# radoslawkrolikowski/financial-market-data-analysis

Measured on NVIDIA H100. Metric: sequences/sec (train step) biGRU h=256 seq=128 feat=64, higher is better.
Workload: dtype bf16x3 (fp32-class: split bf16 operand pairs on tensor cores, fp32 accumulate / state / gradients)

## Files before the change

### financial_market_data_analysis_b200/_lib.py

```python
from __future__ import annotations

import ctypes as C
import os
import threading

_HERE = os.path.dirname(os.path.abspath(__file__))
LIB_PATH = os.path.join(_HERE, "libbigru_b200.so")

PREC_FP32, PREC_BF16, PREC_BF16X3 = 0, 1, 2
SQNORM_WS = 528
LOSS_CE, LOSS_BCE, LOSS_MLSM = 0, 1, 2
ERR_ARG, ERR_CUDA, ERR_DEVICE, ERR_UNSUPPORTED = -1, -2, -3, -4

_vp, _i, _i64, _f, _u64, _d = C.c_void_p, C.c_int, C.c_int64, C.c_float, C.c_uint64, C.c_double

SIGNATURES = {
    "bigru_last_error": (C.c_char_p, []),
    "bigru_version": (_i, []),
    "bigru_device_check": (_i, [_i]),
    "bigru_plan_create": (_i, [_i, _i, _i, _i, _i, _i, _i, _i, C.POINTER(_vp)]),
    "bigru_plan_destroy": (_i, [_vp]),
    "bigru_param_count": (_i64, [_vp]),
    "bigru_param_offset": (_i, [_vp, _i, _i, _i, C.POINTER(_i64), C.POINTER(_i64), C.POINTER(_i64)]),
    "bigru_workspace_bytes": (_i, [_vp, C.POINTER(C.c_size_t), C.POINTER(C.c_size_t)]),
    "bigru_stash_argmax_offset": (_i, [_vp, C.POINTER(C.c_size_t)]),
    "bigru_stash_output_offset": (_i, [_vp, _i, C.POINTER(C.c_size_t)]),
    "bigru_workspace_region": (_i, [_vp, _i, _i, C.POINTER(_i), C.POINTER(C.c_size_t), C.POINTER(C.c_size_t), C.POINTER(_i64)]),
    "bigru_forward": (_i, [_vp, _vp, _vp, _vp, _f, _i, _i, _u64, _vp, _vp, _vp, _vp, _vp]),
    "bigru_backward": (_i, [_vp, _vp, _vp, _vp, _f, _i, _i, _u64, _vp, _vp, _vp, _vp, _vp, _vp, _vp]),
    "bigru_infer_workspace_bytes": (_i, [_vp, C.POINTER(C.c_size_t)]),
    "bigru_infer": (_i, [_vp, _vp, _vp, _vp, _vp, _vp, _vp]),
    "bigru_forward_lengths": (_i, [_vp, _vp, _vp, _vp, _f, _i, _i, _u64, _vp, _vp, _vp, _vp, _vp, _vp]),
    "bigru_backward_lengths": (_i, [_vp, _vp, _vp, _vp, _f, _i, _i, _u64, _vp, _vp, _vp, _vp, _vp, _vp, _vp, _vp]),
    "bigru_infer_lengths": (_i, [_vp, _vp, _vp, _vp, _vp, _vp, _vp, _vp]),
    "bigru_loss": (_i, [_i, _vp, _vp, _vp, _vp, _i, _i, _d, _vp, _vp, _vp]),
    "bigru_sqnorm": (_i, [_vp, _i64, _vp, _vp, _vp]),
    "bigru_adam_tick": (_i, [_vp, _vp, _vp]),
    "bigru_clip_adam_step_dev": (_i, [_vp, _vp, _vp, _vp, _i64, _vp, _f, _f, _f, _f, _f, _vp, _f, _vp]),
    "bigru_launch_count_add": (None, [C.c_longlong]),
    "bigru_window_gather_norm": (_i, [_vp, _vp, _vp, _i64, _i64, _i, _i, _i, _vp, _vp]),
    "bigru_window_targets": (_i, [_vp, _i64, _i64, _i, _i, _i, _vp, _vp]),
    "bigru_multilabel_counts": (_i, [_vp, _vp, _i, _i, _vp, _vp]),
    "bigru_chunk_minmax": (_i, [_vp, _i64, _i, _i64, _i64, _vp, _vp, _vp]),
    "bigru_infer_window": (_i, [_vp, _vp, _vp, _vp, _i, _i, _i, _i, _i, _i, _i, _vp, _vp, _vp]),
    "bigru_window_features": (_i, [_vp, _vp, _vp, _vp, _vp, _i64, C.POINTER(_i), _i, C.POINTER(_i), _i, C.POINTER(_i), _i, _i, _f, _i,
                                   _f, _f, _vp, _vp, C.POINTER(_i), _vp]),
    "bigru_launch_count": (C.c_longlong, []),
    "bigru_prof_enable": (_i, [_i]),
    "bigru_prof_classes": (_i, []),
    "bigru_prof_class_name": (C.c_char_p, [_i]),
    "bigru_prof_report": (_i, [_i, C.POINTER(_d), C.POINTER(C.c_longlong), C.POINTER(_d), C.POINTER(_d)]),
}

_lib = None
_lock = threading.Lock()


def load():
    global _lib
    with _lock:
        if _lib is None:
            if not os.path.exists(LIB_PATH):
                raise RuntimeError(
                    f"{LIB_PATH} is missing: build it with `python -m financial_market_data_analysis_b200.build` "
                    "(or __graft_entry__.build()). This package has no CPU/PyTorch fallback.")
            lib = C.CDLL(LIB_PATH)
            for name, (res, args) in SIGNATURES.items():
                fn = getattr(lib, name)
                fn.restype, fn.argtypes = res, args
            _lib = lib
    return _lib


def check(rc: int, what: str):
    if rc == 0:
        return
    msg = load().bigru_last_error().decode("utf-8", "replace")
    if rc in (ERR_ARG, ERR_UNSUPPORTED):
        raise ValueError(f"{what}: {msg} (code {rc})")
    raise RuntimeError(f"{what}: {msg} (code {rc})")


def ptr(t):
    return None if t is None else C.c_void_p(t.data_ptr())
```

### financial_market_data_analysis_b200/csrc/api.cu

```cuda
#include "common.cuh"
#include "kernels_f32.cuh"
#include "tc_hopper.cuh"
#include "features.cuh"
#include "infer_small.cuh"

#include <cstring>
#include <new>

static thread_local char g_err[512] = "";
void bigru_set_error(const char* fmt, ...) {
    va_list ap;
    va_start(ap, fmt);
    vsnprintf(g_err, sizeof(g_err), fmt, ap);
    va_end(ap);
}

extern "C" const char* bigru_last_error(void) { return g_err; }
extern "C" int bigru_version(void) { return 207; }

extern "C" int bigru_device_check(int dev) {
    int n = 0;
    if (cudaGetDeviceCount(&n) != cudaSuccess || n <= 0 || dev >= n) {
        cudaGetLastError();
        bigru_set_error("no CUDA device %d (libbigru_b200 has no CPU fallback)", dev);
        return BIGRU_ERR_DEVICE;
    }
    cudaDeviceProp p;
    CUDA_TRY(cudaGetDeviceProperties(&p, dev));
    if (p.major != 9 || p.minor != 0) {
        bigru_set_error("device %d is sm_%d%d; libbigru_b200 is built for sm_90a (H100) only", dev, p.major, p.minor);
        return BIGRU_ERR_DEVICE;
    }
    return BIGRU_OK;
}

struct StashF32 {
    int64_t Y[16], G[16], X[16];
    int64_t YP[16], XP[16];
    int64_t cat, arg, total;
};
struct ScratchF32 {
    int64_t gi, gh, dgi, dgh, dYa, dYb, dhc, dcat, csum, dgiP, dghP, tcw, part, total;
};
static inline int64_t in_pitch(const bigru_plan& p, int l) { return rup(p.in_size(l), 8); }
static inline int64_t plane_floats(const bigru_plan& p, int64_t n) {
    return p.prec == BIGRU_PREC_FP32 ? 0 : rup((p.prec == BIGRU_PREC_BF16X3 ? 2 : 1) * n, 128) / 2;
}
static StashF32 stash_layout(const bigru_plan& p) {
    StashF32 s{};
    int64_t o = 0;
    const int64_t BT = (int64_t)p.B * p.T;
    for (int l = 0; l < p.L; ++l) {
        s.Y[l] = o; o += BT * p.D * p.H;
        s.G[l] = o; o += (int64_t)p.D * BT * 4 * p.H;
        s.X[l] = o; o += BT * p.in_size(l);
        o = rup(o, 64);
        s.YP[l] = o; o += plane_floats(p, BT * p.D * p.H);
        s.XP[l] = o; o += plane_floats(p, BT * in_pitch(p, l));
    }
    s.cat = o; o += (int64_t)p.B * 3 * p.H;
    s.arg = o; o += (int64_t)p.B * p.H;
    s.total = o;
    return s;
}
static int64_t dw_part_floats(const bigru_plan& p, int l, int64_t N) {
    const int64_t BT = (int64_t)p.B * p.T, M = 3LL * p.H;
    const int s = wg_splits(cdiv64(M, htc::WG_BM) * cdiv64(N, htc::WG_BN) * p.D, cdiv64(BT, htc::WG_BK));
    return s > 1 ? (int64_t)s * p.D * M * N : 0;
}
static ScratchF32 scratch_layout(const bigru_plan& p) {
    ScratchF32 s{};
    int64_t o = 0;
    const int64_t BT = (int64_t)p.B * p.T;
    const int64_t wide = p.D * p.H > p.F ? p.D * p.H : p.F;
    s.gi = o; o += (int64_t)p.D * BT * 3 * p.H;
    s.gh = o; o += (int64_t)p.D * p.B * 3 * p.H;
    s.dgi = o; o += (int64_t)p.D * BT * 3 * p.H;
    s.dgh = o; o += (int64_t)p.D * BT * 3 * p.H;
    s.dYa = o; o += BT * wide;
    s.dYb = o; o += BT * wide;
    s.dhc = o; o += (int64_t)p.D * p.B * p.H;
    s.dcat = o; o += (int64_t)p.B * 3 * p.H;
    s.csum = o; o += (int64_t)COLSUM_MAX_CHUNKS * (3 * p.H > p.C ? 3 * p.H : p.C);
    o = rup(o, 64);
    s.dgiP = o; o += plane_floats(p, (int64_t)p.D * BT * 3 * p.H);
    s.dghP = o; o += plane_floats(p, (int64_t)p.D * BT * 3 * p.H);
    s.tcw = o;
    s.part = o;
    if (p.prec != BIGRU_PREC_FP32) {
        const int64_t H3 = 3LL * p.H, B = p.B, C = p.C, D = p.D;
        int64_t need = 0, part = 0;
        for (int l = 0; l < p.L; ++l) {
            const int64_t I = p.in_size(l);
            need = std::max(need, tc_pack_elems(H3, I, D, p.prec));
            need = std::max(need, tc_pack_elems(I, H3, D, p.prec));
            part = std::max(part, std::max(dw_part_floats(p, l, I), dw_part_floats(p, l, p.H)));
        }
        const int64_t h[4] = {tc_gemm_ws_elems(B, C, H3, 1, p.prec), tc_gemm_ws_elems(B, H3, C, 1, p.prec),
                              tc_gemm_ws_elems(C, H3, B, 1, p.prec), tc_gemm_ws_elems(H3, p.H, B, 1, p.prec)};
        for (int64_t v : h) need = std::max(need, v);
        o += plane_floats(p, need);
        s.part = o; o += part;
    }
    s.total = o;
    return s;
}
struct InferF32 {
    int64_t gi, gh, y[2], cat, arg, xp, yp[2], tcw, total;
};
static InferF32 infer_layout(const bigru_plan& p) {
    InferF32 s{};
    int64_t o = 0;
    const int64_t BT = (int64_t)p.B * p.T, DH = (int64_t)p.D * p.H;
    const bool tc = p.prec != BIGRU_PREC_FP32;
    s.gi = o; o += (int64_t)p.D * BT * 3 * p.H;
    s.gh = o; if (!tc) o += (int64_t)p.D * p.B * 3 * p.H;
    s.y[0] = o; o += BT * DH;
    s.y[1] = o; if (!tc && p.L > 1) o += BT * DH;
    s.cat = o; o += (int64_t)p.B * 3 * p.H;
    s.arg = o; o += (int64_t)p.B * p.H;
    o = rup(o, 64);
    s.xp = o; o += plane_floats(p, BT * in_pitch(p, 0));
    s.yp[0] = o; if (p.L > 1) o += plane_floats(p, BT * DH);
    s.yp[1] = o; if (p.L > 2) o += plane_floats(p, BT * DH);
    s.tcw = o;
    if (tc) {
        int64_t need = tc_gemm_ws_elems(p.B, p.C, 3LL * p.H, 1, p.prec);
        for (int l = 0; l < p.L; ++l) need = std::max(need, tc_pack_elems(3LL * p.H, p.in_size(l), p.D, p.prec));
        o += plane_floats(p, need);
    }
    s.total = o;
    return s;
}

static int tc_plan_check(const bigru_plan& p) {
    if (p.prec == BIGRU_PREC_BF16X3 && ((p.H != 128 && p.H != 256) || p.B % 32 != 0)) {
        bigru_set_error("BIGRU_PREC_BF16X3 supports hidden_size 128 or 256 and batch %% 32 == 0 (got H=%d B=%d; the Python mirror pads "
                        "other batch sizes with zero rows); use BIGRU_PREC_FP32 for other shapes", p.H, p.B);
        return BIGRU_ERR_UNSUPPORTED;
    }
    if (p.prec == BIGRU_PREC_BF16 && !(((p.H == 128 || p.H == 256) && p.B % 16 == 0) || (p.H == 512 && p.B % 32 == 0))) {
        bigru_set_error("BIGRU_PREC_BF16 supports hidden_size 128 or 256 with batch %% 16 == 0 and hidden_size 512 with batch %% 32 == 0 "
                        "(got H=%d B=%d; the Python mirror pads other batch sizes with zero rows); use BIGRU_PREC_FP32 for other shapes", p.H, p.B);
        return BIGRU_ERR_UNSUPPORTED;
    }
    return BIGRU_OK;
}

static int plan_gemm(const bigru_plan& p, const GemmArgs& g, int cls, htc::bf16_t* tcw, cudaStream_t st) {
    return p.prec == BIGRU_PREC_FP32 ? sgemm_launch(g, st) : tc_gemm_launch(g, p.prec, cls, tcw, st);
}

static Planes plan_planes(const bigru_plan& p, const float* buf, int64_t off, int64_t cols, int64_t rows, int64_t depth,
                          int64_t pitch) {
    const htc::bf16_t* hi = reinterpret_cast<const htc::bf16_t*>(buf + off);
    return Planes{hi, p.prec == BIGRU_PREC_BF16X3 ? hi + depth * rows * pitch : nullptr, cols, rows, depth, pitch};
}
static Planes input_planes(const bigru_plan& p, const float* planes, int l, bool own) {
    const int64_t BT = (int64_t)p.B * p.T;
    return own ? plan_planes(p, planes, 0, p.in_size(l), BT, 1, in_pitch(p, l))
               : plan_planes(p, planes, 0, (int64_t)p.D * p.H, BT, 1, (int64_t)p.D * p.H);
}
static htc::bf16_t* mut(const Planes& q) { return const_cast<htc::bf16_t*>(q.hi); }
static htc::bf16_t* mut_lo(const Planes& q) { return const_cast<htc::bf16_t*>(q.lo); }

extern "C" int bigru_plan_create(int B, int T, int F, int H, int L, int C, int bidirectional, int precision,
                                 bigru_plan** out) {
    if (!out) { bigru_set_error("plan_create: out is null"); return BIGRU_ERR_ARG; }
    if (B <= 0 || T <= 0 || F <= 0 || H <= 0 || L <= 0 || L > 16 || C <= 0) {
        bigru_set_error("plan_create: bad shape B=%d T=%d F=%d H=%d L=%d C=%d", B, T, F, H, L, C);
        return BIGRU_ERR_ARG;
    }
    if (precision != BIGRU_PREC_FP32 && precision != BIGRU_PREC_BF16 && precision != BIGRU_PREC_BF16X3) {
        bigru_set_error("plan_create: unknown precision %d", precision);
        return BIGRU_ERR_ARG;
    }
    bigru_plan* p = new (std::nothrow) bigru_plan();
    if (!p) { bigru_set_error("plan_create: out of host memory"); return BIGRU_ERR_ARG; }
    p->B = B; p->T = T; p->F = F; p->H = H; p->L = L; p->C = C; p->D = bidirectional ? 2 : 1; p->prec = precision;
    p->nparams = p->off_linb() + C;
    if (precision != BIGRU_PREC_FP32) {
        int rc = tc_plan_check(*p);
        if (rc != BIGRU_OK) { delete p; return rc; }
    }
    p->stash_bytes = (size_t)stash_layout(*p).total * sizeof(float);
    p->scratch_bytes = (size_t)scratch_layout(*p).total * sizeof(float);
    *out = p;
    return BIGRU_OK;
}

extern "C" int bigru_plan_destroy(bigru_plan* plan) { delete plan; return BIGRU_OK; }
extern "C" int64_t bigru_param_count(const bigru_plan* plan) { return plan ? plan->nparams : -1; }

extern "C" int bigru_param_offset(const bigru_plan* p, int layer, int dir, int which, int64_t* offset,
                                  int64_t* rows, int64_t* cols) {
    if (!p || !offset || !rows || !cols || layer < 0 || layer > p->L || dir < 0 || dir >= p->D || which < 0 || which > 3) {
        bigru_set_error("param_offset: bad argument");
        return BIGRU_ERR_ARG;
    }
    if (layer == p->L) {
        if (which == 0) { *offset = p->off_linw(); *rows = p->C; *cols = 3 * p->H; }
        else if (which == 2) { *offset = p->off_linb(); *rows = p->C; *cols = 1; }
        else { bigru_set_error("param_offset: linear has which 0 (weight) or 2 (bias)"); return BIGRU_ERR_ARG; }
        return BIGRU_OK;
    }
    switch (which) {
        case 0: *offset = p->off_wih(layer, dir); *rows = 3 * p->H; *cols = p->in_size(layer); break;
        case 1: *offset = p->off_whh(layer, dir); *rows = 3 * p->H; *cols = p->H; break;
        case 2: *offset = p->off_bih(layer, dir); *rows = 3 * p->H; *cols = 1; break;
        default: *offset = p->off_bhh(layer, dir); *rows = 3 * p->H; *cols = 1; break;
    }
    return BIGRU_OK;
}

extern "C" int bigru_workspace_bytes(const bigru_plan* p, size_t* stash_bytes, size_t* scratch_bytes) {
    if (!p || !stash_bytes || !scratch_bytes) { bigru_set_error("workspace_bytes: null argument"); return BIGRU_ERR_ARG; }
    *stash_bytes = p->stash_bytes;
    *scratch_bytes = p->scratch_bytes;
    return BIGRU_OK;
}

extern "C" int bigru_stash_argmax_offset(const bigru_plan* p, size_t* byte_offset) {
    if (!p || !byte_offset) { bigru_set_error("stash_argmax_offset: null argument"); return BIGRU_ERR_ARG; }
    *byte_offset = (size_t)stash_layout(*p).arg * sizeof(float);
    return BIGRU_OK;
}

extern "C" int bigru_stash_output_offset(const bigru_plan* p, int layer, size_t* byte_offset) {
    if (!p || !byte_offset || layer < 0 || layer >= p->L) { bigru_set_error("stash_output_offset: bad argument"); return BIGRU_ERR_ARG; }
    *byte_offset = (size_t)stash_layout(*p).Y[layer] * sizeof(float);
    return BIGRU_OK;
}

extern "C" int bigru_workspace_region(const bigru_plan* p, int which, int layer, int* in_scratch, size_t* byte_offset,
                                      size_t* lo_byte_offset, int64_t* pitch) {
    if (!p || !in_scratch || !byte_offset || !lo_byte_offset || !pitch) {
        bigru_set_error("workspace_region: null argument");
        return BIGRU_ERR_ARG;
    }
    const bool planes = which == BIGRU_WS_Y_PLANES || which == BIGRU_WS_IN_PLANES || which == BIGRU_WS_DGI_PLANES ||
                        which == BIGRU_WS_DGH_PLANES;
    const bool stashed = which == BIGRU_WS_GATES || which == BIGRU_WS_Y_PLANES || which == BIGRU_WS_IN_PLANES;
    const bool layer_ok = stashed ? layer >= 0 && layer < p->L
                        : which == BIGRU_WS_DY ? layer >= 0 && layer < p->L && layer < 2
                        : which == BIGRU_WS_DCAT ? layer == p->L : layer == 0;
    if (which < 0 || which >= BIGRU_WS_COUNT || !layer_ok) {
        bigru_set_error("workspace_region: bad region %d or layer %d", which, layer);
        return BIGRU_ERR_ARG;
    }
    if (planes && p->prec == BIGRU_PREC_FP32) {
        bigru_set_error("workspace_region: BIGRU_PREC_FP32 keeps no bf16 planes");
        return BIGRU_ERR_UNSUPPORTED;
    }
    const StashF32 S = stash_layout(*p);
    const ScratchF32 W = scratch_layout(*p);
    const int64_t BT = (int64_t)p->B * p->T, H3 = 3LL * p->H, DH = (int64_t)p->D * p->H;
    int64_t off = 0, pt = 0, depth_rows = 0;
    switch (which) {
        case BIGRU_WS_GATES:      off = S.G[layer]; pt = 4LL * p->H; break;
        case BIGRU_WS_Y_PLANES:   off = S.YP[layer]; pt = DH; depth_rows = BT; break;
        case BIGRU_WS_IN_PLANES:  off = S.XP[layer]; pt = in_pitch(*p, layer); depth_rows = BT; break;
        case BIGRU_WS_DGI:        off = W.dgi; pt = H3; break;
        case BIGRU_WS_DGH:        off = W.dgh; pt = H3; break;
        case BIGRU_WS_DGI_PLANES: off = W.dgiP; pt = H3; depth_rows = p->D * BT; break;
        case BIGRU_WS_DGH_PLANES: off = W.dghP; pt = H3; depth_rows = p->D * BT; break;
        case BIGRU_WS_DY:         off = (p->L - 1 - layer) % 2 == 0 ? W.dYa : W.dYb; pt = DH; break;
        case BIGRU_WS_DHC:        off = W.dhc; pt = p->H; break;
        default:                  off = W.dcat; pt = H3; break;
    }
    *in_scratch = stashed ? 0 : 1;
    *byte_offset = (size_t)off * sizeof(float);
    *lo_byte_offset = planes && p->prec == BIGRU_PREC_BF16X3 ? *byte_offset + (size_t)(depth_rows * pt) * 2 : SIZE_MAX;
    *pitch = pt;
    return BIGRU_OK;
}

static inline unsigned nblk(int64_t n, int bs) { return (unsigned)cdiv64(n, bs); }

struct FwdBufs {
    float *gi, *gh, *cat, *arg;
    htc::bf16_t* tcw;
    float *X[16], *Y[16], *G[16], *XP[16], *YP[16];
};
static FwdBufs train_bufs(const bigru_plan& p, float* stash, float* scratch) {
    const StashF32 S = stash_layout(p);
    const ScratchF32 W = scratch_layout(p);
    FwdBufs b{};
    b.gi = scratch + W.gi; b.gh = scratch + W.gh; b.cat = stash + S.cat; b.arg = stash + S.arg;
    b.tcw = reinterpret_cast<htc::bf16_t*>(scratch + W.tcw);
    for (int l = 0; l < p.L; ++l) {
        b.X[l] = stash + S.X[l]; b.Y[l] = stash + S.Y[l]; b.G[l] = stash + S.G[l];
        b.XP[l] = stash + S.XP[l]; b.YP[l] = stash + S.YP[l];
    }
    return b;
}
static FwdBufs infer_bufs(const bigru_plan& p, float* ws) {
    const InferF32 I = infer_layout(p);
    const bool tc = p.prec != BIGRU_PREC_FP32;
    FwdBufs b{};
    b.gi = ws + I.gi; b.gh = ws + I.gh; b.cat = ws + I.cat; b.arg = ws + I.arg;
    b.tcw = reinterpret_cast<htc::bf16_t*>(ws + I.tcw);
    b.XP[0] = ws + I.xp;
    for (int l = 0; l < p.L; ++l) {
        const bool top = l == p.L - 1;
        b.Y[l] = !tc ? ws + I.y[l % 2] : top ? ws + I.y[0] : nullptr;
        b.YP[l] = tc && !top ? ws + I.yp[l % 2] : nullptr;
    }
    return b;
}

static int forward_plan(const bigru_plan& p, const float* params, const float* x, const float* h0, const int* len, float drop,
                        int spatial, int training, uint64_t seed, const FwdBufs& buf, float* logits, float* hn,
                        cudaStream_t st) {
    if (len && h0) {
        bigru_set_error("forward: lengths together with an initial hidden state are not supported");
        return BIGRU_ERR_UNSUPPORTED;
    }
    if (p.prec == BIGRU_PREC_BF16 && h0) {
        bigru_set_error("BIGRU_PREC_BF16: an initial hidden state is not supported; use BIGRU_PREC_FP32 or BIGRU_PREC_BF16X3");
        return BIGRU_ERR_UNSUPPORTED;
    }
    const int B = p.B, T = p.T, H = p.H, D = p.D;
    const int64_t BT = (int64_t)B * T;
    const bool do_drop = training && drop > 0.f;
    const float* inp = x;
    for (int l = 0; l < p.L; ++l) {
        const int I = (int)p.in_size(l);
        if (do_drop && (l == 0 || p.L > 1)) {
            float* xd = buf.X[l];
            KLAUNCH(KC_MISC, 0.0, 0.0, st, dropout_kernel<<<132 * 8, 256, 0, st>>>(inp, xd, BT * I, T, I, l == 0 ? spatial : 0, drop, seed, (uint32_t)l));
            inp = xd;
        }
        float* Y = buf.Y[l];
        float* G = buf.G[l];
        const float* h0l = h0 ? h0 + (int64_t)l * D * B * H : nullptr;
        float* hnl = hn ? hn + (int64_t)l * D * B * H : nullptr;
        if (p.prec != BIGRU_PREC_FP32) {
            const bool own = l == 0 || do_drop;
            const Planes xp = input_planes(p, own ? buf.XP[l] : buf.YP[l - 1], l, own);
            if (own)
                KLAUNCH(KC_PACK, 0.0, 0.0, st, htc::to_planes_kernel<<<132 * 8, 256, 0, st>>>(inp, BT, I, (int)xp.pitch, mut(xp), mut_lo(xp)));
            Planes wp;
            TRY(tc_pack(params + p.off_wih(l, 0), I, 1, p.ld_block(l), 3 * H, I, D, p.prec, buf.tcw, &wp, st));
            {
                ProfScope ps(KC_TC_GEMM, 2.0 * BT * 3 * H * (double)I * D, 0.0, st);
                htc::WgJob j = wg_job(buf.gi, (int)BT, 3 * H, 3 * H, D, cdiv64(I, htc::WG_BK));
                j.bias = params + p.off_bih(l, 0); j.zBias = p.ld_block(l); j.zC = BT * 3 * H;
                j.b.zsel = 1;
                TRY(wg_gemm(j, xp, false, wp, false, p.prec, st));
            }
            htc::bf16_t *yh = nullptr, *yl = nullptr;
            if (buf.YP[l]) {
                const Planes yp = plan_planes(p, buf.YP[l], 0, (int64_t)D * H, BT, 1, (int64_t)D * H);
                yh = mut(yp); yl = mut_lo(yp);
            }
            TRY(tc_scan_fwd(p, l, buf.gi, params + p.off_whh(l, 0), params + p.off_bhh(l, 0), h0l, Y, G, hnl, yh, yl, len, st));
            inp = Y;
            continue;
        }
        GemmArgs g = gemm_args(inp, params + p.off_wih(l, 0), buf.gi, (int)BT, 3 * H, I, I, 1, I, 1, 3 * H);
        g.bias = params + p.off_bih(l, 0);
        g.batch = D; g.zA = 0; g.zB = p.ld_block(l); g.zBias = p.ld_block(l); g.zC = BT * 3 * H;
        TRY(plan_gemm(p, g, KC_TC_GEMM, buf.tcw, st));
        for (int s = 0; s < T; ++s) {
            const float* hp; int64_t sam, zA;
            if (s == 0) { hp = h0l; sam = H; zA = (int64_t)B * H; }
            else {
                hp = Y + (int64_t)(s - 1) * D * H;
                sam = (int64_t)T * D * H;
                zA = D == 2 ? ((int64_t)(T - s) - (s - 1)) * D * H + H : 0;
            }
            GemmArgs r = gemm_args(hp, params + p.off_whh(l, 0), buf.gh, B, 3 * H, hp ? H : 0, sam, 1, H, 1, 3 * H);
            r.bias = params + p.off_bhh(l, 0);
            r.batch = D; r.zA = zA; r.zB = p.ld_block(l); r.zBias = p.ld_block(l); r.zC = (int64_t)B * 3 * H;
            if (hp) { TRY(sgemm_launch(r, st)); }
            else {
                r.A = params; r.K = 1; r.sam = 0; r.sak = 1; r.zA = 0;
                r.mask_period = 1; r.mask_skip = 0;
                TRY(sgemm_launch(r, st));
            }
            KLAUNCH(KC_GATES_FWD, 0.0, 0.0, st, gru_gates_fwd_kernel<<<nblk((int64_t)D * B * H, 256), 256, 0, st>>>(buf.gi, buf.gh, h0l, Y, G,
                                                                              hnl, B, T, H, D, s, len));
        }
        inp = Y;
    }
    KLAUNCH(KC_HEAD, 0.0, 0.0, st, head_pool_kernel<<<nblk((int64_t)B * H, 128), 128, 0, st>>>(buf.Y[p.L - 1], buf.cat, (int*)buf.arg, B, T, H, D, len));
    GemmArgs lin = gemm_args(buf.cat, params + p.off_linw(), logits, B, p.C, 3 * H, 3 * H, 1, 3 * H, 1, p.C);
    lin.bias = params + p.off_linb();
    TRY(plan_gemm(p, lin, KC_HEAD, buf.tcw, st));
    return BIGRU_OK;
}

static int backward_plan(const bigru_plan& p, const float* params, const float* x, const float* h0, const int* len, float drop,
                         int spatial, int training, uint64_t seed, const float* stash, float* scratch,
                         const float* dlogits, float* grads, float* dx, float* dh0, cudaStream_t st) {
    if (len && (h0 || dh0)) {
        bigru_set_error("backward: lengths together with an initial hidden state or its gradient are not supported");
        return BIGRU_ERR_UNSUPPORTED;
    }
    if (p.prec == BIGRU_PREC_BF16 && (h0 || dh0)) {
        bigru_set_error("BIGRU_PREC_BF16: initial hidden state / its gradient are not supported");
        return BIGRU_ERR_UNSUPPORTED;
    }
    const StashF32 S = stash_layout(p);
    const ScratchF32 W = scratch_layout(p);
    const int B = p.B, T = p.T, H = p.H, D = p.D, C = p.C;
    const int64_t BT = (int64_t)B * T, H3 = 3LL * H;
    const bool do_drop = training && drop > 0.f;
    const bool tc = p.prec != BIGRU_PREC_FP32;
    float* dhc = scratch + W.dhc;
    htc::bf16_t* tcw = reinterpret_cast<htc::bf16_t*>(scratch + W.tcw);
    CUDA_TRY(cudaMemsetAsync(grads, 0, sizeof(float) * p.nparams, st));
    GemmArgs a = gemm_args(dlogits, params + p.off_linw(), scratch + W.dcat, B, 3 * H, C, C, 1, 1, 3 * H, 3 * H);
    TRY(plan_gemm(p, a, KC_HEAD, tcw, st));
    GemmArgs w = gemm_args(dlogits, stash + S.cat, grads + p.off_linw(), C, 3 * H, B, 1, C, 1, 3 * H, 3 * H);
    TRY(plan_gemm(p, w, KC_HEAD, tcw, st));
    TRY(colsum_launch(dlogits, grads + p.off_linb(), B, C, C, 1, 0, 0, scratch + W.csum, st));
    KLAUNCH(KC_HEAD, 0.0, 0.0, st, head_bwd_dy_kernel<<<nblk(BT * H, 256), 256, 0, st>>>(scratch + W.dcat, (const int*)(stash + S.arg), scratch + W.dYa, dhc, B, T, H, D, len));
    for (int l = p.L - 1; l >= 0; --l) {
        const int I = (int)p.in_size(l);
        const bool even = (p.L - 1 - l) % 2 == 0;
        const bool drop_l = do_drop && (l == 0 || p.L > 1);
        float* dY = scratch + (even ? W.dYa : W.dYb);
        float* dYnext = scratch + (even ? W.dYb : W.dYa);
        const float* Y = stash + S.Y[l];
        const float* G = stash + S.G[l];
        const float* h0l = h0 ? h0 + (int64_t)l * D * B * H : nullptr;
        float* dgi = scratch + W.dgi;
        float* dgh = scratch + W.dgh;
        if (l != p.L - 1) CUDA_TRY(cudaMemsetAsync(dhc, 0, sizeof(float) * D * B * H, st));
        const Planes gip = plan_planes(p, scratch, W.dgiP, H3, BT, D, H3);
        const Planes ghp = plan_planes(p, scratch, W.dghP, H3, BT, D, H3);
        if (tc) {
            TRY(tc_scan_bwd(p, l, G, Y, h0l, dY, dhc, dgi, dgh, params + p.off_whh(l, 0), mut(gip), mut_lo(gip), mut(ghp), mut_lo(ghp), len, st));
        } else {
            for (int s = 0; s < T; ++s) {
                KLAUNCH(KC_GATES_BWD, 0.0, 0.0, st, gru_gates_bwd_kernel<<<nblk((int64_t)D * B * H, 256), 256, 0, st>>>(G, Y, h0l, dY, dhc, dgi, dgh, B, T, H, D, s, len));
                const int t0 = T - 1 - s, t1 = s;
                GemmArgs r = gemm_args(dgh + (int64_t)t0 * 3 * H, params + p.off_whh(l, 0), dhc, B, H, 3 * H,
                                       (int64_t)T * 3 * H, 1, 1, H, H);
                r.beta = 1; r.batch = D;
                r.zA = BT * 3 * H + (int64_t)(t1 - t0) * 3 * H; r.zB = p.ld_block(l); r.zC = (int64_t)B * H;
                TRY(sgemm_launch(r, st));
            }
        }
        if (dh0) CUDA_TRY(cudaMemcpyAsync(dh0 + (int64_t)l * D * B * H, dhc, sizeof(float) * D * B * H,
                                          cudaMemcpyDeviceToDevice, st));
        if (tc) {
            const int64_t kb = cdiv64(BT, htc::WG_BK);
            float* part = scratch + W.part;
            {
                ProfScope ps(KC_TC_GEMM_DWIH, 2.0 * H3 * I * (double)BT * D, 0.0, st);
                htc::WgJob j = wg_job(grads + p.off_wih(l, 0), (int)H3, I, I, D, kb);
                j.zC = p.ld_block(l); j.a.zsel = 1; j.part = part;
                j.splits = wg_splits(cdiv64(H3, htc::WG_BM) * cdiv64(I, htc::WG_BN) * D, kb);
                const bool own = l == 0 || do_drop;
                TRY(wg_gemm(j, gip, true, input_planes(p, stash + (own ? S.XP[l] : S.YP[l - 1]), l, own), true, p.prec, st));
            }
            if (T > 1) {
                ProfScope ps(KC_TC_GEMM_DWHH, 2.0 * H3 * H * (double)BT * D, 0.0, st);
                htc::WgJob j = wg_job(grads + p.off_whh(l, 0), (int)H3, H, H, D, kb);
                j.zC = p.ld_block(l); j.a.zsel = 1; j.part = part;
                j.b.coff = H; j.b.kshift[0] = -1; j.b.kshift[1] = 1;
                j.splits = wg_splits(cdiv64(H3, htc::WG_BM) * cdiv64(H, htc::WG_BN) * D, kb);
                TRY(wg_gemm(j, ghp, true, plan_planes(p, stash, S.YP[l], (int64_t)D * H, BT, 1, (int64_t)D * H), true, p.prec, st));
            }
        } else {
            const float* inp = drop_l ? stash + S.X[l] : l == 0 ? x : stash + S.Y[l - 1];
            const int splitk = (int)min((int64_t)64, max((int64_t)1, BT / 512));
            for (int d = 0; d < D; ++d) {
                const float* dgi_d = dgi + (int64_t)d * BT * 3 * H;
                const float* dgh_d = dgh + (int64_t)d * BT * 3 * H;
                GemmArgs wi = gemm_args(dgi_d, inp, grads + p.off_wih(l, d), 3 * H, I, (int)BT, 1, 3 * H, 1, I, I);
                wi.splitk = splitk;
                TRY(sgemm_launch(wi, st));
                if (T > 1) {
                    const float* hp = Y + (int64_t)d * H + (d == 0 ? -(int64_t)D * H : (int64_t)D * H);
                    GemmArgs wh = gemm_args(dgh_d, hp, grads + p.off_whh(l, d), 3 * H, H, (int)BT, 1, 3 * H, 1,
                                            (int64_t)D * H, H);
                    wh.splitk = splitk; wh.mask_period = T; wh.mask_skip = d == 0 ? 0 : T - 1;
                    TRY(sgemm_launch(wh, st));
                }
            }
        }
        for (int d = 0; d < D; ++d) {
            const float* dgi_d = dgi + (int64_t)d * BT * 3 * H;
            const float* dgh_d = dgh + (int64_t)d * BT * 3 * H;
            if (h0l) {
                const int tf = d == 0 ? 0 : T - 1;
                GemmArgs w0 = gemm_args(dgh_d + (int64_t)tf * 3 * H, h0l + (int64_t)d * B * H, grads + p.off_whh(l, d),
                                        3 * H, H, B, 1, (int64_t)T * 3 * H, 1, H, H);
                w0.beta = 1;
                TRY(plan_gemm(p, w0, KC_TC_GEMM_DWHH, tcw, st));
            }
            TRY(colsum_launch(dgi_d, grads + p.off_bih(l, d), BT, 3 * H, 3 * H, 1, 0, 0, scratch + W.csum, st));
            TRY(colsum_launch(dgh_d, grads + p.off_bhh(l, d), BT, 3 * H, 3 * H, 1, 0, 0, scratch + W.csum, st));
        }
        float* dxo = l == 0 ? dx : dYnext;
        if (!dxo) continue;
        if (tc) {
            Planes wp;
            TRY(tc_pack(params + p.off_wih(l, 0), 1, I, p.ld_block(l), I, 3 * H, D, p.prec, tcw, &wp, st));
            ProfScope ps(KC_TC_GEMM_DX, 2.0 * BT * I * (double)H3 * D, 0.0, st);
            htc::WgJob j = wg_job(dxo, (int)BT, I, I, 1, D * (H3 / htc::WG_BK));
            j.kbd = (int)(H3 / htc::WG_BK); j.kcat = 1; j.a.zsel = 1; j.b.zsel = 1;
            TRY(wg_gemm(j, gip, false, wp, false, p.prec, st));
        } else {
            for (int d = 0; d < D; ++d) {
                GemmArgs gx = gemm_args(dgi + (int64_t)d * BT * 3 * H, params + p.off_wih(l, d), dxo, (int)BT, I, 3 * H,
                                        3 * H, 1, 1, I, I);
                gx.beta = d;
                TRY(sgemm_launch(gx, st));
            }
        }
        if (drop_l)
            KLAUNCH(KC_MISC, 0.0, 0.0, st, dropout_kernel<<<132 * 8, 256, 0, st>>>(dxo, dxo, BT * I, T, I, l == 0 ? spatial : 0, drop, seed, (uint32_t)l));
    }
    return BIGRU_OK;
}

extern "C" int bigru_forward(const bigru_plan* plan, const float* d_params, const float* d_x, const float* d_h0,
                             float dropout_p, int spatial, int training, uint64_t seed, void* d_stash,
                             void* d_scratch, float* d_logits, float* d_hn, void* stream) {
    return bigru_forward_lengths(plan, d_params, d_x, d_h0, dropout_p, spatial, training, seed, d_stash, d_scratch, d_logits,
                                 d_hn, nullptr, stream);
}

extern "C" int bigru_forward_lengths(const bigru_plan* plan, const float* d_params, const float* d_x, const float* d_h0,
                                     float dropout_p, int spatial, int training, uint64_t seed, void* d_stash,
                                     void* d_scratch, float* d_logits, float* d_hn, const int32_t* d_lengths, void* stream) {
    if (!plan || !d_params || !d_x || !d_stash || !d_scratch || !d_logits) {
        bigru_set_error("forward: null argument");
        return BIGRU_ERR_ARG;
    }
    if (dropout_p < 0.f || dropout_p >= 1.f) { bigru_set_error("forward: dropout_p must be in [0,1)"); return BIGRU_ERR_ARG; }
    return forward_plan(*plan, d_params, d_x, d_h0, d_lengths, dropout_p, spatial, training, seed,
                        train_bufs(*plan, (float*)d_stash, (float*)d_scratch), d_logits, d_hn, (cudaStream_t)stream);
}

extern "C" int bigru_infer_workspace_bytes(const bigru_plan* p, size_t* bytes) {
    if (!p || !bytes) { bigru_set_error("infer_workspace_bytes: null argument"); return BIGRU_ERR_ARG; }
    *bytes = (size_t)infer_layout(*p).total * sizeof(float);
    return BIGRU_OK;
}

extern "C" int bigru_infer(const bigru_plan* plan, const float* d_params, const float* d_x, const float* d_h0,
                           void* d_workspace, float* d_logits, void* stream) {
    return bigru_infer_lengths(plan, d_params, d_x, d_h0, d_workspace, d_logits, nullptr, stream);
}

extern "C" int bigru_infer_lengths(const bigru_plan* plan, const float* d_params, const float* d_x, const float* d_h0,
                                   void* d_workspace, float* d_logits, const int32_t* d_lengths, void* stream) {
    if (!plan || !d_params || !d_x || !d_workspace || !d_logits) {
        bigru_set_error("infer: null argument");
        return BIGRU_ERR_ARG;
    }
    return forward_plan(*plan, d_params, d_x, d_h0, d_lengths, 0.f, 0, 0, 0, infer_bufs(*plan, (float*)d_workspace), d_logits,
                        nullptr, (cudaStream_t)stream);
}

extern "C" int bigru_backward(const bigru_plan* plan, const float* d_params, const float* d_x, const float* d_h0,
                              float dropout_p, int spatial, int training, uint64_t seed, const void* d_stash,
                              void* d_scratch, const float* d_dlogits, float* d_grads, float* d_dx, float* d_dh0,
                              void* stream) {
    return bigru_backward_lengths(plan, d_params, d_x, d_h0, dropout_p, spatial, training, seed, d_stash, d_scratch, d_dlogits,
                                  d_grads, d_dx, d_dh0, nullptr, stream);
}

extern "C" int bigru_backward_lengths(const bigru_plan* plan, const float* d_params, const float* d_x, const float* d_h0,
                                      float dropout_p, int spatial, int training, uint64_t seed, const void* d_stash,
                                      void* d_scratch, const float* d_dlogits, float* d_grads, float* d_dx, float* d_dh0,
                                      const int32_t* d_lengths, void* stream) {
    if (!plan || !d_params || !d_x || !d_stash || !d_scratch || !d_dlogits || !d_grads) {
        bigru_set_error("backward: null argument");
        return BIGRU_ERR_ARG;
    }
    return backward_plan(*plan, d_params, d_x, d_h0, d_lengths, dropout_p, spatial, training, seed, (const float*)d_stash,
                         (float*)d_scratch, d_dlogits, d_grads, d_dx, d_dh0, (cudaStream_t)stream);
}

extern "C" int bigru_chunk_minmax(const float* d_table, int64_t N, int F, int64_t row_lo, int64_t row_hi, float* d_min,
                                  float* d_max, void* stream) {
    if (!d_table || !d_min || !d_max || F <= 0 || row_lo < 0 || row_hi > N || row_lo >= row_hi) {
        bigru_set_error("chunk_minmax: bad argument");
        return BIGRU_ERR_ARG;
    }
    KLAUNCH(KC_GATHER, 0.0, 4.0 * (row_hi - row_lo) * F, (cudaStream_t)stream,
            chunk_minmax_kernel<<<(F + 31) / 32, dim3(32, 8), 0, (cudaStream_t)stream>>>(d_table, F, row_lo, row_hi, d_min, d_max));
    return BIGRU_OK;
}

extern "C" int bigru_window_features(const float* d_close, const float* d_high, const float* d_low, const float* d_volume,
                                     const float* d_delta, int64_t n, const int* vol_periods, int n_vol, const int* price_periods,
                                     int n_price, const int* delta_periods, int n_delta, int bb_period, float bb_std, int stochastic,
                                     float n1, float n2, float* d_out, float* d_targets, int* n_out, void* stream) {
    if (n_vol < 0 || n_vol > 8 || n_price < 0 || n_price > 8 || n_delta < 0 || n_delta > 8 || bb_period < 0 || n < 0 ||
        (n_vol && !vol_periods) || (n_price && !price_periods) || (n_delta && !delta_periods)) {
        bigru_set_error("window_features: bad argument (at most 8 periods per list)");
        return BIGRU_ERR_ARG;
    }
    FeatureCfg cfg{};
    cfg.n_vol = n_vol; cfg.n_price = n_price; cfg.n_delta = n_delta;
    for (int i = 0; i < n_vol; ++i) cfg.vol_p[i] = vol_periods[i];
    for (int i = 0; i < n_price; ++i) cfg.price_p[i] = price_periods[i];
    for (int i = 0; i < n_delta; ++i) cfg.delta_p[i] = delta_periods[i];
    for (int i = 0; i < 8; ++i)
        if ((i < n_vol && cfg.vol_p[i] < 1) || (i < n_price && cfg.price_p[i] < 1) || (i < n_delta && cfg.delta_p[i] < 1)) {
            bigru_set_error("window_features: periods must be >= 1");
            return BIGRU_ERR_ARG;
        }
    cfg.bb_period = bb_period; cfg.bb_std = bb_std; cfg.stochastic = stochastic ? 1 : 0; cfg.n1 = n1; cfg.n2 = n2;
    cfg.n_out = (bb_period > 0 ? 2 : 0) + n_vol + n_price + n_delta + (stochastic ? 1 : 0) + 2;
    if (n_out) *n_out = cfg.n_out;
    if (!d_out || n == 0) return BIGRU_OK;
    if (!d_close || !d_high || !d_low || (n_vol && !d_volume) || (n_delta && !d_delta)) {
        bigru_set_error("window_features: null column");
        return BIGRU_ERR_ARG;
    }
    int halo = 14;
    for (int i = 0; i < n_vol; ++i) halo = std::max(halo, cfg.vol_p[i] - 1);
    for (int i = 0; i < n_price; ++i) halo = std::max(halo, cfg.price_p[i] - 1);
    for (int i = 0; i < n_delta; ++i) halo = std::max(halo, cfg.delta_p[i] - 1);
    halo = std::max(halo, bb_period - 1);
    if (halo > 4095) { bigru_set_error("window_features: periods above 4096 rows are not supported"); return BIGRU_ERR_UNSUPPORTED; }
    const int span = FEAT_TR + halo;
    const size_t smem = sizeof(float) * ((size_t)4 * span + 16 + (size_t)FEAT_TR * (cfg.n_out + 4));
    const bool fast = n_vol == 2 && cfg.vol_p[0] == 6 && cfg.vol_p[1] == 20 && n_price == 1 && cfg.price_p[0] == 20 && n_delta == 1 &&
                      cfg.delta_p[0] == 12 && bb_period == 20 && stochastic;
    if (smem > 48 * 1024)
        CUDA_TRY(fast ? cudaFuncSetAttribute(window_features_kernel<true>, cudaFuncAttributeMaxDynamicSharedMemorySize, (int)smem)
                      : cudaFuncSetAttribute(window_features_kernel<false>, cudaFuncAttributeMaxDynamicSharedMemorySize, (int)smem));
    const unsigned blocks = (unsigned)std::min<int64_t>((n + FEAT_TR - 1) / FEAT_TR, 132 * 8);
    if (fast)
        KLAUNCH(KC_GATHER, 0.0, 4.0 * n * (5 + cfg.n_out + 4), (cudaStream_t)stream,
                window_features_kernel<true><<<blocks, FEAT_TR, smem, (cudaStream_t)stream>>>(d_close, d_high, d_low, d_volume, d_delta, n, cfg,
                                                                                              halo, d_out, d_targets));
    else
        KLAUNCH(KC_GATHER, 0.0, 4.0 * n * (5 + cfg.n_out + 4), (cudaStream_t)stream,
                window_features_kernel<false><<<blocks, FEAT_TR, smem, (cudaStream_t)stream>>>(d_close, d_high, d_low, d_volume, d_delta, n, cfg,
                                                                                               halo, d_out, d_targets));
    return BIGRU_OK;
}

extern "C" int bigru_infer_window(const float* d_params, const float* d_x, const float* d_xmin, const float* d_xmax, int B, int T,
                                  int F, int H, int L, int C, int bidirectional, float* d_logits, float* d_probs, void* stream) {
    if (!d_params || !d_x || !d_logits || B <= 0 || T <= 0 || F <= 0 || H <= 0 || L <= 0 || C <= 0 || ((d_xmin == nullptr) != (d_xmax == nullptr))) {
        bigru_set_error("infer_window: bad argument");
        return BIGRU_ERR_ARG;
    }
    const int D = bidirectional ? 2 : 1, DH = D * H, W = F > DH ? F : DH;
    const size_t smem = sizeof(float) * ((size_t)T * W + (size_t)T * DH + 2 * (size_t)DH + 3 * (size_t)H);
    if (DH > 1024 || smem > 200 * 1024) {
        bigru_set_error("infer_window: window too large for the single-CTA path (D*H=%d, %zu bytes of shared memory); use bigru_forward", DH, smem);
        return BIGRU_ERR_UNSUPPORTED;
    }
    if (smem > 48 * 1024)
        CUDA_TRY(cudaFuncSetAttribute(infer_window_kernel, cudaFuncAttributeMaxDynamicSharedMemorySize, (int)smem));
    const int threads = std::max(32, ((DH + 31) / 32) * 32);
    KLAUNCH(KC_MISC, 0.0, 0.0, (cudaStream_t)stream,
            infer_window_kernel<<<B, threads, smem, (cudaStream_t)stream>>>(d_params, d_x, d_xmin, d_xmax, T, F, H, L, C, D, d_logits, d_probs));
    return BIGRU_OK;
}

extern "C" int bigru_loss(int kind, const float* d_logits, const void* d_target, const float* d_weight,
                          const float* d_pos_weight, int B, int C, double denom, float* d_loss, float* d_dlogits,
                          void* stream) {
    if (!d_logits || !d_target || !d_loss || B <= 0 || C <= 0 || denom <= 0 || kind < 0 || kind > 2) {
        bigru_set_error("loss: bad argument");
        return BIGRU_ERR_ARG;
    }
    cudaStream_t st = (cudaStream_t)stream;
    CUDA_TRY(cudaMemsetAsync(d_loss, 0, sizeof(float), st));
    if (kind == BIGRU_LOSS_MLSM) { d_weight = nullptr; d_pos_weight = nullptr; }
    KLAUNCH(KC_LOSS, 0.0, 0.0, st, loss_kernel<<<1, 256, 0, st>>>(kind, d_logits, d_target, d_weight, d_pos_weight, B, C,
                                             (float)(1.0 / denom), d_loss, d_dlogits));
    return BIGRU_OK;
}

extern "C" int bigru_sqnorm(const float* d_g, int64_t n, float* d_out, float* d_ws, void* stream) {
    if (!d_g || !d_out || !d_ws || n < 0) { bigru_set_error("sqnorm: bad argument"); return BIGRU_ERR_ARG; }
    if (n == 0) return BIGRU_OK;
    const int blocks = (int)min((int64_t)BIGRU_SQNORM_WS, cdiv64(n, 256));
    KLAUNCH(KC_OPTIM, 0.0, 0.0, (cudaStream_t)stream, sqnorm_kernel<<<blocks, 256, 0, (cudaStream_t)stream>>>(d_g, n, d_ws));
    KLAUNCH(KC_OPTIM, 0.0, 0.0, (cudaStream_t)stream, sqnorm_finish_kernel<<<1, 32, 0, (cudaStream_t)stream>>>(d_ws, blocks, d_out));
    return BIGRU_OK;
}

extern "C" int bigru_adam_tick(int* d_step, float* d_sqnorm, void* stream) {
    if (!d_step || !d_sqnorm) { bigru_set_error("adam_tick: null argument"); return BIGRU_ERR_ARG; }
    KLAUNCH(KC_OPTIM, 0.0, 0.0, (cudaStream_t)stream, adam_tick_kernel<<<1, 32, 0, (cudaStream_t)stream>>>(d_step, d_sqnorm));
    return BIGRU_OK;
}

extern "C" int bigru_clip_adam_step_dev(float* d_params, float* d_grads, float* d_m, float* d_v, int64_t n,
                                        const float* d_sqnorm, float clip, float lr, float b1, float b2, float eps,
                                        const int* d_step, float grad_scale, void* stream) {
    if (!d_params || !d_grads || !d_m || !d_v || !d_sqnorm || !d_step || n <= 0) {
        bigru_set_error("clip_adam_step_dev: bad argument");
        return BIGRU_ERR_ARG;
    }
    const unsigned blocks = (unsigned)min((int64_t)132 * 8, cdiv64(n, 256));
    KLAUNCH(KC_OPTIM, 0.0, 0.0, (cudaStream_t)stream, clip_adam_dev_kernel<<<blocks, 256, 0, (cudaStream_t)stream>>>(d_params, d_grads, d_m, d_v, n, d_sqnorm, clip,
                                                                    lr, b1, b2, eps, d_step, grad_scale));
    return BIGRU_OK;
}

extern "C" int bigru_window_gather_norm(const float* d_src, const float* d_xmin, const float* d_xmax, int64_t start,
                                        int64_t N, int B, int T, int F, float* d_out, void* stream) {
    if (B == 0 && T > 0 && F > 0 && start >= 0) return BIGRU_OK;
    if (!d_src || !d_out || B < 0 || T <= 0 || F <= 0 || start < 0 || (B > 0 && start + B + T - 1 > N) ||
        ((d_xmin == nullptr) != (d_xmax == nullptr))) {
        bigru_set_error("window_gather_norm: bad argument (start=%lld B=%d T=%d N=%lld)", (long long)start, B, T, (long long)N);
        return BIGRU_ERR_ARG;
    }
    cudaStream_t st = (cudaStream_t)stream;
    const bool vec = F % 4 == 0 && ((uintptr_t)d_src % 16 == 0) && ((uintptr_t)d_out % 16 == 0) &&
                     (!d_xmin || (((uintptr_t)d_xmin % 16 == 0) && ((uintptr_t)d_xmax % 16 == 0)));
    const int64_t total = (int64_t)B * T * (vec ? F / 4 : F);
    const unsigned blocks = (unsigned)min((int64_t)132 * 16, cdiv64(total, 256));
    const double bytes = 4.0 * ((double)B * T * F + (double)(B + T - 1) * F);
    if (vec) KLAUNCH(KC_GATHER, 0.0, bytes, st, window_gather_kernel<4><<<blocks, 256, 0, st>>>(d_src, d_xmin, d_xmax, start, B, T, F, d_out));
    else KLAUNCH(KC_GATHER, 0.0, bytes, st, window_gather_kernel<1><<<blocks, 256, 0, st>>>(d_src, d_xmin, d_xmax, start, B, T, F, d_out));
    return BIGRU_OK;
}

extern "C" int bigru_window_targets(const float* d_y, int64_t start, int64_t N, int B, int T, int C, float* d_out,
                                    void* stream) {
    if (B == 0 && T > 0 && C > 0 && start >= 0) return BIGRU_OK;
    if (!d_y || !d_out || B < 0 || T <= 0 || C <= 0 || start < 0 || (B > 0 && start + B + T - 1 > N)) {
        bigru_set_error("window_targets: bad argument");
        return BIGRU_ERR_ARG;
    }
    if (B == 0) return BIGRU_OK;
    KLAUNCH(KC_GATHER, 0.0, 0.0, (cudaStream_t)stream, window_targets_kernel<<<nblk((int64_t)B * C, 256), 256, 0, (cudaStream_t)stream>>>(d_y, start, B, T, C, d_out));
    return BIGRU_OK;
}

extern "C" int bigru_multilabel_counts(const float* d_logits, const float* d_target, int B, int C,
                                       long long* d_counts, void* stream) {
    if (!d_logits || !d_target || !d_counts || B <= 0 || C <= 0) { bigru_set_error("multilabel_counts: bad argument"); return BIGRU_ERR_ARG; }
    KLAUNCH(KC_MISC, 0.0, 0.0, (cudaStream_t)stream, multilabel_counts_kernel<<<nblk(B, 128), 128, 0, (cudaStream_t)stream>>>(d_logits, d_target, B, C,
                                                                            (unsigned long long*)d_counts));
    return BIGRU_OK;
}

extern "C" long long bigru_launch_count(void) { return profiler().launches.load(); }
extern "C" void bigru_launch_count_add(long long n) { profiler().launches.fetch_add(n, std::memory_order_relaxed); }

extern "C" int bigru_prof_enable(int on) {
    Profiler& p = profiler();
    std::lock_guard<std::mutex> g(p.mu);
    for (auto& r : p.recs) { cudaEventDestroy(r.a); cudaEventDestroy(r.b); }
    p.recs.clear();
    p.enabled.store(on ? 1 : 0);
    return BIGRU_OK;
}

extern "C" int bigru_prof_classes(void) { return KC_COUNT; }
extern "C" const char* bigru_prof_class_name(int cls) { return cls >= 0 && cls < KC_COUNT ? kKClassNames[cls] : ""; }

extern "C" int bigru_prof_report(int cls, double* ms, long long* launches, double* flops, double* bytes) {
    if (cls < 0 || cls >= KC_COUNT || !ms || !launches || !flops || !bytes) { bigru_set_error("prof_report: bad argument"); return BIGRU_ERR_ARG; }
    Profiler& p = profiler();
    std::lock_guard<std::mutex> g(p.mu);
    *ms = 0; *launches = 0; *flops = 0; *bytes = 0;
    for (auto& r : p.recs) {
        if (r.cls != cls) continue;
        CUDA_TRY(cudaEventSynchronize(r.b));
        float t = 0.f;
        CUDA_TRY(cudaEventElapsedTime(&t, r.a, r.b));
        *ms += t; *launches += 1; *flops += r.flops; *bytes += r.bytes;
    }
    return BIGRU_OK;
}
```

### financial_market_data_analysis_b200/csrc/tc_hopper.cuh

```cuda
#pragma once
#include "common.cuh"
#include "kernels_f32.cuh"
#include <algorithm>
#include <cuda.h>
#include <cuda_bf16.h>

namespace htc {

typedef __nv_bfloat16 bf16_t;

__device__ __forceinline__ uint32_t smem_u32(const void* p) { return (uint32_t)__cvta_generic_to_shared(p); }

__device__ __forceinline__ void split_bf16(float x, bf16_t& hi, bf16_t& lo) {
    hi = __float2bfloat16(x);
    lo = __float2bfloat16(x - __bfloat162float(hi));
}

__device__ __forceinline__ void ldsm_x4(uint32_t addr, uint32_t (&r)[4]) {
    asm volatile("ldmatrix.sync.aligned.m8n8.x4.shared.b16 {%0, %1, %2, %3}, [%4];"
                 : "=r"(r[0]), "=r"(r[1]), "=r"(r[2]), "=r"(r[3]) : "r"(addr));
}
__device__ __forceinline__ void ldsm_x2(uint32_t addr, uint32_t (&r)[2]) {
    asm volatile("ldmatrix.sync.aligned.m8n8.x2.shared.b16 {%0, %1}, [%2];" : "=r"(r[0]), "=r"(r[1]) : "r"(addr));
}
__device__ __forceinline__ void mma_bf16(float (&c)[4], const uint32_t (&a)[4], uint32_t b0, uint32_t b1) {
    asm volatile("mma.sync.aligned.m16n8k16.row.col.f32.bf16.bf16.f32 {%0, %1, %2, %3}, {%4, %5, %6, %7}, {%8, %9}, "
                 "{%0, %1, %2, %3};"
                 : "+f"(c[0]), "+f"(c[1]), "+f"(c[2]), "+f"(c[3])
                 : "r"(a[0]), "r"(a[1]), "r"(a[2]), "r"(a[3]), "r"(b0), "r"(b1));
}

template <int PITCH>
__device__ __forceinline__ uint32_t swz(int row, int k) {
    return (uint32_t)(row * PITCH + ((((k >> 3) ^ (row & 7))) << 4) + ((k & 7) << 1));
}

__device__ __forceinline__ uint32_t mapa(uint32_t local_addr, uint32_t cta) {
    uint32_t r;
    asm volatile("mapa.shared::cluster.u32 %0, %1, %2;" : "=r"(r) : "r"(local_addr), "r"(cta));
    return r;
}
__device__ __forceinline__ void st_cluster_v2_f32(uint32_t addr, float2 v) {
    asm volatile("st.shared::cluster.v2.f32 [%0], {%1, %2};" ::"r"(addr), "f"(v.x), "f"(v.y) : "memory");
}
__device__ __forceinline__ void cluster_arrive() { asm volatile("barrier.cluster.arrive.release;" ::: "memory"); }
__device__ __forceinline__ void cluster_wait() { asm volatile("barrier.cluster.wait.acquire;" ::: "memory"); }
__device__ __forceinline__ uint32_t cluster_rank() {
    uint32_t r;
    asm volatile("mov.u32 %0, %%cluster_ctarank;" : "=r"(r));
    return r;
}

constexpr int WG_BM = 128, WG_BN = 128, WG_BK = 64;

__global__ void tc_pack_kernel(const float* __restrict__ src, int64_t s_r, int64_t s_k, int64_t zsrc, int R, int K, int Rp, int Kp,
                               bf16_t* __restrict__ hi, bf16_t* __restrict__ lo) {
    __shared__ float tile[32][33];
    const int z = blockIdx.z, r0 = blockIdx.y * 32, k0 = blockIdx.x * 32;
    const float* a = src + z * zsrc;
    const bool kfast = s_k == 1;
    for (int j = threadIdx.y; j < 32; j += 8) {
        const int r = r0 + (kfast ? j : threadIdx.x), k = k0 + (kfast ? threadIdx.x : j);
        float v = 0.f;
        if (r < R && k < K) v = a[(int64_t)r * s_r + (int64_t)k * s_k];
        if (kfast) tile[j][threadIdx.x] = v; else tile[threadIdx.x][j] = v;
    }
    __syncthreads();
    for (int j = threadIdx.y; j < 32; j += 8) {
        const int r = r0 + j, k = k0 + threadIdx.x;
        const int64_t o = ((int64_t)z * Rp + r) * Kp + k;
        bf16_t h, l;
        split_bf16(tile[j][threadIdx.x], h, l);
        hi[o] = h;
        if (lo) lo[o] = l;
    }
}

__global__ void to_planes_kernel(const float* __restrict__ src, int64_t rows, int cols, int pitch, bf16_t* __restrict__ hi,
                                 bf16_t* __restrict__ lo) {
    const int64_t n = rows * cols;
    for (int64_t i = (int64_t)blockIdx.x * blockDim.x + threadIdx.x; i < n; i += (int64_t)gridDim.x * blockDim.x) {
        const int64_t r = i / cols, c = i % cols, o = r * pitch + c;
        bf16_t h, l;
        split_bf16(src[i], h, l);
        hi[o] = h;
        if (lo) lo[o] = l;
    }
}

__device__ __forceinline__ void mbar_init(uint64_t* bar, uint32_t count) {
    asm volatile("mbarrier.init.shared::cta.b64 [%0], %1;" ::"r"(smem_u32(bar)), "r"(count) : "memory");
}
__device__ __forceinline__ void mbar_arrive_expect_tx(uint64_t* bar, uint32_t bytes) {
    asm volatile("mbarrier.arrive.expect_tx.shared::cta.b64 _, [%0], %1;" ::"r"(smem_u32(bar)), "r"(bytes) : "memory");
}
__device__ __forceinline__ void mbar_arrive(uint64_t* bar) {
    asm volatile("mbarrier.arrive.shared::cta.b64 _, [%0];" ::"r"(smem_u32(bar)) : "memory");
}
__device__ __forceinline__ bool mbar_try_wait(uint64_t* bar, uint32_t parity) {
    uint32_t ok;
    asm volatile(
        "{\n\t.reg .pred p;\n\t"
        "mbarrier.try_wait.parity.shared::cta.b64 p, [%1], %2;\n\t"
        "selp.u32 %0, 1, 0, p;\n\t}" : "=r"(ok) : "r"(smem_u32(bar)), "r"(parity) : "memory");
    return ok != 0;
}
__device__ __forceinline__ bool mbar_try_wait_cluster(uint64_t* bar, uint32_t parity) {
    uint32_t ok;
    asm volatile(
        "{\n\t.reg .pred p;\n\t"
        "mbarrier.try_wait.parity.acquire.cluster.shared::cta.b64 p, [%1], %2;\n\t"
        "selp.u32 %0, 1, 0, p;\n\t}" : "=r"(ok) : "r"(smem_u32(bar)), "r"(parity) : "memory");
    return ok != 0;
}
template <bool CLUSTER = false>
__device__ __forceinline__ void mbar_wait(uint64_t* bar, uint32_t parity) {
    auto ready = [&] { return CLUSTER ? mbar_try_wait_cluster(bar, parity) : mbar_try_wait(bar, parity); };
    if (ready()) return;
    uint64_t t0, t;
    asm volatile("mov.u64 %0, %%globaltimer;" : "=l"(t0));
    for (uint32_t i = 0;; ++i) {
        if (ready()) return;
        if ((i & 1023u) == 1023u) {
            asm volatile("mov.u64 %0, %%globaltimer;" : "=l"(t));
            if (t - t0 > 5000000000ull) __trap();
        }
    }
}
__device__ __forceinline__ void bulk_copy_to_peer(uint32_t src, uint32_t bytes, uint64_t* bar, uint32_t cta) {
    asm volatile("cp.async.bulk.shared::cluster.shared::cta.mbarrier::complete_tx::bytes [%0], [%1], %2, [%3];"
                 ::"r"(mapa(src, cta)), "r"(src), "r"(bytes), "r"(mapa(smem_u32(bar), cta)) : "memory");
}
__device__ __forceinline__ void tma_load_3d(uint32_t dst, const CUtensorMap* m, uint64_t* bar, int c0, int c1, int c2) {
    asm volatile("cp.async.bulk.tensor.3d.shared::cluster.global.mbarrier::complete_tx::bytes [%0], [%1, {%3, %4, %5}], [%2];"
                 ::"r"(dst), "l"(reinterpret_cast<uint64_t>(m)), "r"(smem_u32(bar)), "r"(c0), "r"(c1), "r"(c2) : "memory");
}
__device__ __forceinline__ uint64_t wg_desc(uint32_t saddr, uint32_t lbo) {
    return (uint64_t)((saddr & 0x3FFFF) >> 4) | ((uint64_t)(lbo >> 4) << 16) | ((uint64_t)(1024 >> 4) << 32) | ((uint64_t)1 << 62);
}
template <int TA, int TB>
__device__ __forceinline__ void wgmma_m64n128k16(float (&d)[64], uint64_t da, uint64_t db) {
    asm volatile("wgmma.mma_async.sync.aligned.m64n128k16.f32.bf16.bf16 {%0, %1, %2, %3, %4, %5, %6, %7, %8, %9, %10, %11, %12, %13, %14, %15, %16, %17, %18, %19, %20, %21, %22, %23, %24, %25, %26, %27, %28, %29, %30, %31, %32, %33, %34, %35, %36, %37, %38, %39, %40, %41, %42, %43, %44, %45, %46, %47, %48, %49, %50, %51, %52, %53, %54, %55, %56, %57, %58, %59, %60, %61, %62, %63}, %64, %65, 1, 1, 1, %66, %67;"
                 : "+f"(d[0]), "+f"(d[1]), "+f"(d[2]), "+f"(d[3]), "+f"(d[4]), "+f"(d[5]), "+f"(d[6]), "+f"(d[7]), "+f"(d[8]), "+f"(d[9]), "+f"(d[10]), "+f"(d[11]), "+f"(d[12]), "+f"(d[13]), "+f"(d[14]), "+f"(d[15]), "+f"(d[16]), "+f"(d[17]), "+f"(d[18]), "+f"(d[19]), "+f"(d[20]), "+f"(d[21]), "+f"(d[22]), "+f"(d[23]), "+f"(d[24]), "+f"(d[25]), "+f"(d[26]), "+f"(d[27]), "+f"(d[28]), "+f"(d[29]), "+f"(d[30]), "+f"(d[31]), "+f"(d[32]), "+f"(d[33]), "+f"(d[34]), "+f"(d[35]), "+f"(d[36]), "+f"(d[37]), "+f"(d[38]), "+f"(d[39]), "+f"(d[40]), "+f"(d[41]), "+f"(d[42]), "+f"(d[43]), "+f"(d[44]), "+f"(d[45]), "+f"(d[46]), "+f"(d[47]), "+f"(d[48]), "+f"(d[49]), "+f"(d[50]), "+f"(d[51]), "+f"(d[52]), "+f"(d[53]), "+f"(d[54]), "+f"(d[55]), "+f"(d[56]), "+f"(d[57]), "+f"(d[58]), "+f"(d[59]), "+f"(d[60]), "+f"(d[61]), "+f"(d[62]), "+f"(d[63])
                 : "l"(da), "l"(db), "n"(TA), "n"(TB));
}

struct WgOp {
    int zsel, coff, kshift[2];
};
struct WgJob {
    WgOp a, b;
    float* C; const float* bias; float* part;
    int M, N, tm, tn, batch, splits;
    int kblocks, kbd;
    int kcat;
    int beta;
    int64_t ldc, zC, zBias;
};

template <int NS, int STAGES, int AMN, int BMN>
__global__ void __launch_bounds__(384, 1)
wg_gemm_kernel(const __grid_constant__ CUtensorMap ta_hi, const __grid_constant__ CUtensorMap ta_lo,
               const __grid_constant__ CUtensorMap tb_hi, const __grid_constant__ CUtensorMap tb_lo, const WgJob j) {
    constexpr int NH = NS == 1 ? 1 : 2;
    constexpr int PLANE = WG_BM * WG_BK * 2;
    constexpr int STAGE = 2 * NH * PLANE;
    extern __shared__ __align__(1024) uint8_t wg_smem_raw[];
    uint8_t* sm = reinterpret_cast<uint8_t*>((reinterpret_cast<uintptr_t>(wg_smem_raw) + 1023) & ~(uintptr_t)1023);
    uint64_t* full = reinterpret_cast<uint64_t*>(sm + STAGES * STAGE);
    uint64_t* empty = full + STAGES;
    const int wgi = threadIdx.x / 128, tid = threadIdx.x % 128;
    const int units = j.tm * j.tn * j.batch * j.splits;
    const int per = (j.kblocks + j.splits - 1) / j.splits;
    if (threadIdx.x == 0) {
        for (int i = 0; i < STAGES; ++i) { mbar_init(full + i, 1); mbar_init(empty + i, 2); }
        asm volatile("fence.mbarrier_init.release.cluster;" ::: "memory");
    }
    __syncthreads();
    auto decode = [&](int u, int& s, int& zb, int& m0, int& n0) {
        s = u % j.splits; u /= j.splits;
        n0 = (u % j.tn) * WG_BN; u /= j.tn;
        m0 = (u % j.tm) * WG_BM; zb = u / j.tm;
    };

    if (wgi == 0) {
        if (tid == 0) {
            uint32_t it = 0;
            for (int u = blockIdx.x; u < units; u += gridDim.x) {
                int s, zb, m0, n0;
                decode(u, s, zb, m0, n0);
                const int kb1 = min(j.kblocks, (s + 1) * per);
                for (int kb = s * per; kb < kb1; ++kb, ++it) {
                    const int st = it % STAGES;
                    if (it >= STAGES) mbar_wait(empty + st, ((it / STAGES) - 1) & 1);
                    const uint32_t base = smem_u32(sm + st * STAGE);
                    mbar_arrive_expect_tx(full + st, STAGE);
                    const int dz = j.kcat ? kb / j.kbd : zb, kc = (j.kcat ? kb % j.kbd : kb) * WG_BK;
#pragma unroll
                    for (int h = 0; h < NH; ++h) {
                        const CUtensorMap* ma = h ? &ta_lo : &ta_hi;
                        const CUtensorMap* mb = h ? &tb_lo : &tb_hi;
                        const uint32_t da = base + h * PLANE, db = base + (NH + h) * PLANE;
                        if (AMN) {
                            const int k = kc + (dz ? j.a.kshift[1] : j.a.kshift[0]), r = m0 + dz * j.a.coff;
                            tma_load_3d(da, ma, full + st, r, k, dz * j.a.zsel);
                            tma_load_3d(da + PLANE / 2, ma, full + st, r + 64, k, dz * j.a.zsel);
                        } else {
                            tma_load_3d(da, ma, full + st, kc, m0, dz * j.a.zsel);
                        }
                        if (BMN) {
                            const int k = kc + (dz ? j.b.kshift[1] : j.b.kshift[0]), r = n0 + dz * j.b.coff;
                            tma_load_3d(db, mb, full + st, r, k, dz * j.b.zsel);
                            tma_load_3d(db + PLANE / 2, mb, full + st, r + 64, k, dz * j.b.zsel);
                        } else {
                            tma_load_3d(db, mb, full + st, kc, n0, dz * j.b.zsel);
                        }
                    }
                }
            }
        }
        return;
    }
    const int cg = wgi - 1;
    const int w = tid / 32, l = tid % 32;
    constexpr uint32_t AKS = AMN ? 2048 : 32, BKS = BMN ? 2048 : 32;
    constexpr uint32_t ALBO = AMN ? PLANE / 2 : 16, BLBO = BMN ? PLANE / 2 : 16;
    uint32_t it = 0;
    for (int u = blockIdx.x; u < units; u += gridDim.x) {
        int s, zb, m0, n0;
        decode(u, s, zb, m0, n0);
        const int kb1 = min(j.kblocks, (s + 1) * per);
        float d[64];
#pragma unroll
        for (int i = 0; i < 64; ++i) d[i] = 0.f;
        int prev = -1;
        for (int kb = s * per; kb < kb1; ++kb, ++it) {
            const int st = it % STAGES;
            mbar_wait(full + st, (it / STAGES) & 1);
            const uint32_t base = smem_u32(sm + st * STAGE);
            const uint32_t a_hi = base + cg * (PLANE / 2), a_lo = a_hi + PLANE;
            const uint32_t b_hi = base + NH * PLANE, b_lo = b_hi + PLANE;
            asm volatile("wgmma.fence.sync.aligned;" ::: "memory");
#pragma unroll
            for (int ks = 0; ks < WG_BK / 16; ++ks) {
                wgmma_m64n128k16<AMN, BMN>(d, wg_desc(a_hi + ks * AKS, ALBO), wg_desc(b_hi + ks * BKS, BLBO));
                if (NS != 1) {
                    wgmma_m64n128k16<AMN, BMN>(d, wg_desc(a_hi + ks * AKS, ALBO), wg_desc(b_lo + ks * BKS, BLBO));
                    wgmma_m64n128k16<AMN, BMN>(d, wg_desc(a_lo + ks * AKS, ALBO), wg_desc(b_hi + ks * BKS, BLBO));
                }
            }
            asm volatile("wgmma.commit_group.sync.aligned;" ::: "memory");
            asm volatile("wgmma.wait_group.sync.aligned 1;" ::: "memory");
            if (prev >= 0 && tid == 0) mbar_arrive(empty + prev);
            prev = st;
        }
        asm volatile("wgmma.wait_group.sync.aligned 0;" ::: "memory");
        if (prev >= 0 && tid == 0) mbar_arrive(empty + prev);
        float* C;
        int64_t ldc;
        const float* bias = nullptr;
        if (j.splits > 1) {
            C = j.part + ((int64_t)s * j.batch + zb) * j.M * j.N;
            ldc = j.N;
        } else {
            C = j.C + zb * j.zC;
            ldc = j.ldc;
            if (j.bias) bias = j.bias + zb * j.zBias;
        }
#pragma unroll
        for (int i = 0; i < 16; ++i)
#pragma unroll
            for (int e = 0; e < 4; ++e) {
                const int gm = m0 + cg * 64 + w * 16 + (l >> 2) + (e >= 2 ? 8 : 0);
                const int gn = n0 + 8 * i + 2 * (l & 3) + (e & 1);
                if (gm >= j.M || gn >= j.N) continue;
                float v = d[4 * i + e];
                if (bias) v += bias[gn];
                float* c = C + (int64_t)gm * ldc + gn;
                if (j.beta && j.splits == 1) *c += v;
                else *c = v;
            }
    }
}

__global__ void splitk_reduce_kernel(const float* __restrict__ part, int splits, int batch, int M, int N, float* __restrict__ C,
                                     int64_t ldc, int64_t zC, int beta) {
    const int64_t per = (int64_t)M * N, n = per * batch;
    for (int64_t i = (int64_t)blockIdx.x * blockDim.x + threadIdx.x; i < n; i += (int64_t)gridDim.x * blockDim.x) {
        float v = 0.f;
        for (int s = 0; s < splits; ++s) v += part[(int64_t)s * n + i];
        const int64_t z = i / per, r = i % per;
        float* c = C + z * zC + (r / N) * ldc + r % N;
        *c = beta ? *c + v : v;
    }
}

constexpr int SCAN_U = 64, SCAN_NB = 16, SCAN_THREADS = 256;
constexpr int SCAN_Y = 1, SCAN_G = 2, SCAN_PLANES = 4;
constexpr int SCAN_TRAIN = SCAN_Y | SCAN_G | SCAN_PLANES, SCAN_INFER_LOWER = SCAN_PLANES, SCAN_INFER_TOP = SCAN_Y;

template <int H, int NS>
struct FwdSmem {
    static constexpr int NH = NS == 1 ? 1 : 2;
    static constexpr int WP = H * 2;
    static constexpr int WBYTES = 3 * SCAN_U * WP;
    static constexpr int HBYTES = SCAN_NB * H * 2;
    static constexpr int SLICE = SCAN_NB * SCAN_U * 2;
    static constexpr int TOTAL = NH * WBYTES + 2 * NH * HBYTES + 2 * 8;
};

__device__ __forceinline__ uint32_t hsw(int b, int k) {
    return (uint32_t)((k / SCAN_U) * (SCAN_NB * SCAN_U * 2)) + swz<SCAN_U * 2>(b, k % SCAN_U);
}

template <int H, int NS, int OUT, bool LEN>
__global__ void __launch_bounds__(SCAN_THREADS, 1)
gru_scan_fwd_kernel(const float* __restrict__ gi, const float* __restrict__ Whh, const float* __restrict__ bhh, int64_t zW,
                    const float* __restrict__ h0, float* __restrict__ Y, float* __restrict__ G, float* __restrict__ hn_out,
                    bf16_t* __restrict__ yh, bf16_t* __restrict__ yl, int B, int T, int D, const int* __restrict__ lens) {
    using S = FwdSmem<H, NS>;
    constexpr int U = SCAN_U, CS = H / U, NH = S::NH;
    static_assert(SCAN_THREADS % (SCAN_NB * (U / 8)) == 0, "a thread copies the same Y plane row in every pass");
    extern __shared__ __align__(128) uint8_t smem[];
    uint8_t* Wsm = smem;
    uint8_t* Hsm = smem + NH * S::WBYTES;
    uint64_t* full = reinterpret_cast<uint64_t*>(Hsm + 2 * NH * S::HBYTES);
    const int c = (int)cluster_rank(), tile = blockIdx.y, d = blockIdx.z;
    const int tid = threadIdx.x, lane = tid & 31, warp = tid >> 5;
    const int bt0 = tile * SCAN_NB;
    const float* W = Whh + d * zW;

    for (int i = tid; i < 3 * U * H; i += SCAN_THREADS) {
        const int q = i / H, k = i % H, gte = q / U, u = q % U;
        const float v = W[(int64_t)(gte * H + c * U + u) * H + k];
        bf16_t hi, lo;
        split_bf16(v, hi, lo);
        *reinterpret_cast<bf16_t*>(Wsm + swz<S::WP>(q, k)) = hi;
        if (NH == 2) *reinterpret_cast<bf16_t*>(Wsm + S::WBYTES + swz<S::WP>(q, k)) = lo;
    }
    for (int i = tid; i < SCAN_NB * H; i += SCAN_THREADS) {
        const int b = i / H, k = i % H;
        const float v = h0 ? h0[((int64_t)d * B + bt0 + b) * H + k] : 0.f;
        bf16_t hi, lo;
        split_bf16(v, hi, lo);
        *reinterpret_cast<bf16_t*>(Hsm + hsw(b, k)) = hi;
        if (NH == 2) *reinterpret_cast<bf16_t*>(Hsm + S::HBYTES + hsw(b, k)) = lo;
    }
    if (tid == 0) {
        mbar_init(full, 1);
        mbar_init(full + 1, 1);
        asm volatile("fence.mbarrier_init.release.cluster;" ::: "memory");
    }

    const int ug = warp >> 1, nt = warp & 1;
    int unit[2], bcol[2];
    unit[0] = ug * 16 + (lane >> 2); unit[1] = unit[0] + 8;
    bcol[0] = nt * 8 + 2 * (lane & 3); bcol[1] = bcol[0] + 1;
    float bias[3][2], hp[4];
#pragma unroll
    for (int gte = 0; gte < 3; ++gte)
#pragma unroll
        for (int j = 0; j < 2; ++j) bias[gte][j] = bhh[d * zW + gte * H + c * U + unit[j]];
#pragma unroll
    for (int e = 0; e < 4; ++e) {
        const int b = bt0 + bcol[e & 1], j = c * U + unit[e >> 1];
        hp[e] = h0 ? h0[((int64_t)d * B + b) * H + j] : 0.f;
    }
    int len[2] = {T, T}, rlen = T;
    if (LEN) {
        len[0] = lens[bt0 + bcol[0]]; len[1] = lens[bt0 + bcol[1]];
        rlen = lens[bt0 + (tid / (U / 8)) % SCAN_NB];
    }
    cluster_arrive();
    cluster_wait();

    const int DH = D * H;
    for (int s = 0; s < T; ++s) {
        const int t = d == 0 ? s : T - 1 - s;
        const int buf = s & 1;
        if (s > 0) mbar_wait<true>(full + buf, ((s - 1) >> 1) & 1);
        if (tid == 0 && s + 1 < T) mbar_arrive_expect_tx(full + (buf ^ 1), (CS - 1) * NH * S::SLICE);
        float giv[3][4];
#pragma unroll
        for (int e = 0; e < 4; ++e) {
            const int64_t row = (int64_t)(bt0 + bcol[e & 1]) * T + t;
            const float* gr = gi + ((int64_t)d * B * T + row) * 3 * H + c * U + unit[e >> 1];
#pragma unroll
            for (int gte = 0; gte < 3; ++gte) giv[gte][e] = gr[gte * H];
        }
        float acc[3][4];
#pragma unroll
        for (int gte = 0; gte < 3; ++gte)
#pragma unroll
            for (int e = 0; e < 4; ++e) acc[gte][e] = 0.f;
        const uint32_t hbase = smem_u32(Hsm + buf * NH * S::HBYTES);
        const uint32_t wbase = smem_u32(Wsm);
#pragma unroll 4
        for (int ks = 0; ks < H / 16; ++ks) {
            uint32_t bh[NH][2];
            const int brow = nt * 8 + (lane & 7), bk = ks * 16 + ((lane >> 3) & 1) * 8;
#pragma unroll
            for (int h = 0; h < NH; ++h) ldsm_x2(hbase + h * S::HBYTES + hsw(brow, bk), bh[h]);
#pragma unroll
            for (int gte = 0; gte < 3; ++gte) {
                const int arow = gte * U + ug * 16 + (lane & 15), ak = ks * 16 + (lane >> 4) * 8;
                uint32_t a[NH][4];
#pragma unroll
                for (int h = 0; h < NH; ++h) ldsm_x4(wbase + h * S::WBYTES + swz<S::WP>(arow, ak), a[h]);
                if (NS != 1) {
                    mma_bf16(acc[gte], a[0], bh[NH - 1][0], bh[NH - 1][1]);
                    mma_bf16(acc[gte], a[NH - 1], bh[0][0], bh[0][1]);
                }
                mma_bf16(acc[gte], a[0], bh[0][0], bh[0][1]);
            }
        }
        const int nbuf = buf ^ 1;
#pragma unroll
        for (int e = 0; e < 4; ++e) {
            const int b = bt0 + bcol[e & 1], ul = unit[e >> 1], j = c * U + ul;
            const float r = sigmoid_f(giv[0][e] + acc[0][e] + bias[0][e >> 1]);
            const float z = sigmoid_f(giv[1][e] + acc[1][e] + bias[1][e >> 1]);
            const float hnv = acc[2][e] + bias[2][e >> 1];
            const float n = tanhf(giv[2][e] + r * hnv);
            const bool pad = LEN && t >= len[e & 1];
            const float h = pad ? hp[e] : (1.f - z) * n + z * hp[e];
            hp[e] = h;
            const int64_t row = (int64_t)b * T + t;
            if (OUT & SCAN_Y) Y[row * DH + d * H + j] = pad ? 0.f : h;
            if ((OUT & SCAN_G) && !pad) {
                float* gs = G + ((int64_t)d * B * T + row) * 4 * H + j;
                gs[0] = r; gs[H] = z; gs[2 * H] = n; gs[3 * H] = hnv;
            }
            if (hn_out && s == T - 1) hn_out[((int64_t)d * B + b) * H + j] = h;
            bf16_t hi, lo;
            split_bf16(h, hi, lo);
            uint8_t* la = Hsm + nbuf * NH * S::HBYTES + hsw(bcol[e & 1], j);
            *reinterpret_cast<bf16_t*>(la) = hi;
            if (NH == 2) *reinterpret_cast<bf16_t*>(la + S::HBYTES) = lo;
        }
        asm volatile("fence.proxy.async.shared::cta;" ::: "memory");
        __syncthreads();
        const uint32_t own = smem_u32(Hsm + nbuf * NH * S::HBYTES + c * S::SLICE);
        if (tid == 0 && s + 1 < T) {
#pragma unroll
            for (int p = 1; p < CS; ++p) {
                const uint32_t dst = (c + p) % CS;
#pragma unroll
                for (int h = 0; h < NH; ++h) bulk_copy_to_peer(own + h * S::HBYTES, S::SLICE, full + nbuf, dst);
            }
        }
        if (OUT & SCAN_PLANES) {
            for (int i = tid; i < NH * SCAN_NB * (U / 8); i += SCAN_THREADS) {
                const int h = i / (SCAN_NB * U / 8), r = (i / (U / 8)) % SCAN_NB, kl = (i % (U / 8)) * 8;
                uint4 v = *reinterpret_cast<const uint4*>(Hsm + nbuf * NH * S::HBYTES + h * S::HBYTES + c * S::SLICE +
                                                          swz<U * 2>(r, kl));
                if (LEN && t >= rlen) v = make_uint4(0u, 0u, 0u, 0u);
                *reinterpret_cast<uint4*>((h ? yl : yh) + ((int64_t)(bt0 + r) * T + t) * DH + d * H + c * U + kl) = v;
            }
        }
    }
    cluster_arrive();
    cluster_wait();
}

template <int H, int NS>
struct BwdSmem {
    static constexpr int NH = NS == 1 ? 1 : 2;
    static constexpr int Q = 3 * SCAN_U;
    static constexpr int WP = Q * 2;
    static constexpr int WBYTES = H * WP;
    static constexpr int DBYTES = SCAN_NB * Q * 2;
    static constexpr int SLOT = SCAN_NB * SCAN_U * 4;
    static constexpr int TOTAL = NH * WBYTES + NH * DBYTES + (H / SCAN_U - 1) * SLOT;
    static_assert(NH * DBYTES >= SLOT, "own partial sums alias the dgh tile");
};

__device__ __forceinline__ int xslot(int kl, int b) {
    static_assert(SCAN_NB == 16, "eight column pairs per unit");
    const int g = ((kl >> 1) & 1) * 4 + ((kl >> 2) & 3);
    return kl * SCAN_NB + (((b >> 1) ^ g) << 1) + (b & 1);
}

template <int H, int NS, bool LEN>
__global__ void __launch_bounds__(SCAN_THREADS, 1)
gru_scan_bwd_kernel(const float* __restrict__ G, const float* __restrict__ Y, const float* __restrict__ h0,
                    const float* __restrict__ dY, float* __restrict__ dhc, float* __restrict__ dgi, float* __restrict__ dgh,
                    const float* __restrict__ Whh, int64_t zW, bf16_t* __restrict__ gih, bf16_t* __restrict__ gil,
                    bf16_t* __restrict__ ghh, bf16_t* __restrict__ ghl, int B, int T, int D, const int* __restrict__ lens) {
    using S = BwdSmem<H, NS>;
    constexpr int U = SCAN_U, CS = H / U, NH = S::NH, Q = S::Q, NB = SCAN_NB;
    constexpr int MT = H / 16 / 8;
    constexpr int PAIRS = NB * U / SCAN_THREADS;
    extern __shared__ __align__(128) uint8_t smem[];
    uint8_t* Wsm = smem;
    uint8_t* Dsm = smem + NH * S::WBYTES;
    float* recv = reinterpret_cast<float*>(Dsm + NH * S::DBYTES);
    const int c = (int)cluster_rank(), tile = blockIdx.y, d = blockIdx.z;
    const int tid = threadIdx.x, lane = tid & 31, warp = tid >> 5;
    const int bt0 = tile * NB;
    const float* W = Whh + d * zW;
    float* own = reinterpret_cast<float*>(Dsm);
    auto slot = [&](int src) -> float* { return src == c ? own : recv + (src < c ? src : src - 1) * NB * U; };

    for (int i = tid; i < Q * H; i += SCAN_THREADS) {
        const int q = i / H, k = i % H, gte = q / U, u = q % U;
        const float v = W[(int64_t)(gte * H + c * U + u) * H + k];
        bf16_t hi, lo;
        split_bf16(v, hi, lo);
        *reinterpret_cast<bf16_t*>(Wsm + swz<S::WP>(k, q)) = hi;
        if (NH == 2) *reinterpret_cast<bf16_t*>(Wsm + S::WBYTES + swz<S::WP>(k, q)) = lo;
    }
    float dhr[PAIRS], dhz[PAIRS];
    int plen[PAIRS];
#pragma unroll
    for (int i = 0; i < PAIRS; ++i) {
        const int p = tid + i * SCAN_THREADS, u = p % U, b = p / U;
        dhr[i] = dhc[((int64_t)d * B + bt0 + b) * H + c * U + u];
        dhz[i] = 0.f;
        plen[i] = LEN ? lens[bt0 + b] : T;
    }
    cluster_arrive();
    cluster_wait();

    const int DH = D * H;
    float gr[PAIRS], gz[PAIRS], gn[PAIRS], ghn[PAIRS], hprev[PAIRS], dyv[PAIRS];
    auto load_step = [&](int s) {
        const int t = d == 0 ? T - 1 - s : s;
        const bool first = d == 0 ? t == 0 : t == T - 1;
#pragma unroll
        for (int i = 0; i < PAIRS; ++i) {
            const int p = tid + i * SCAN_THREADS, u = p % U, b = bt0 + p / U, j = c * U + u;
            const int64_t row = (int64_t)b * T + t;
            const float* gs = G + ((int64_t)d * B * T + row) * 4 * H + j;
            gr[i] = gs[0]; gz[i] = gs[H]; gn[i] = gs[2 * H]; ghn[i] = gs[3 * H];
            if (first) hprev[i] = h0 ? h0[((int64_t)d * B + b) * H + j] : 0.f;
            else hprev[i] = Y[((int64_t)b * T + (d == 0 ? t - 1 : t + 1)) * DH + d * H + j];
            dyv[i] = dY[row * DH + d * H + j];
        }
    };
    load_step(0);
    for (int s = 0; s < T; ++s) {
        const int t = d == 0 ? T - 1 - s : s;
        const bool first = d == 0 ? t == 0 : t == T - 1;
        if (s > 0) {
#pragma unroll
            for (int i = 0; i < PAIRS; ++i) {
                const int p = tid + i * SCAN_THREADS, x = xslot(p % U, p / U);
                float v = dhz[i];
#pragma unroll
                for (int src = 0; src < CS; ++src) v += slot(src)[x];
                dhr[i] = v;
            }
        }
        cluster_arrive();
        __syncthreads();
#pragma unroll
        for (int i = 0; i < PAIRS; ++i) {
            const int p = tid + i * SCAN_THREADS, u = p % U, bl = p / U, b = bt0 + bl, j = c * U + u;
            const int64_t row = (int64_t)b * T + t;
            const float r = gr[i], z = gz[i], n = gn[i], hnv = ghn[i], hpv = hprev[i];
            const float dh = dhr[i] + dyv[i];
            float dan = dh * (1.f - z) * (1.f - n * n);
            float dar = dan * hnv * r * (1.f - r);
            float daz = dh * (hpv - n) * z * (1.f - z);
            float dgn = dan * r;
            const bool pad = LEN && t >= plen[i];
            if (pad) dan = dar = daz = dgn = 0.f;
            float* a = dgi + ((int64_t)d * B * T + row) * 3 * H + j;
            float* cg = dgh + ((int64_t)d * B * T + row) * 3 * H + j;
            a[0] = dar; a[H] = daz; a[2 * H] = dan;
            cg[0] = dar; cg[H] = daz; cg[2 * H] = dgn;
            dhz[i] = pad ? dhr[i] : dh * z;
            const float gv[3] = {dar, daz, dgn};
#pragma unroll
            for (int gte = 0; gte < 3; ++gte) {
                bf16_t hi, lo;
                split_bf16(gv[gte], hi, lo);
                *reinterpret_cast<bf16_t*>(Dsm + swz<S::WP>(bl, gte * U + u)) = hi;
                if (NH == 2) *reinterpret_cast<bf16_t*>(Dsm + S::DBYTES + swz<S::WP>(bl, gte * U + u)) = lo;
            }
            bf16_t hi, lo;
            split_bf16(dan, hi, lo);
            const int64_t po = ((int64_t)d * B * T + row) * 3 * H + 2 * H + j;
            gih[po] = hi;
            if (NH == 2) gil[po] = lo;
        }
        if (NS == 1 && s + 1 < T) load_step(s + 1);
        __syncthreads();
        for (int i = tid; i < NH * NB * (Q / 8); i += SCAN_THREADS) {
            const int h = i / (NB * Q / 8), r = (i / (Q / 8)) % NB, q = (i % (Q / 8)) * 8, gte = q / U;
            uint4 v = *reinterpret_cast<const uint4*>(Dsm + h * S::DBYTES + swz<S::WP>(r, q));
            const int64_t o = ((int64_t)d * B * T + (int64_t)(bt0 + r) * T + t) * 3 * H + gte * H + c * U + q % U;
            if (gte < 2) *reinterpret_cast<uint4*>((h ? gil : gih) + o) = v;
            if (first) v = make_uint4(0u, 0u, 0u, 0u);
            *reinterpret_cast<uint4*>((h ? ghl : ghh) + o) = v;
        }
        float acc[MT][2][4];
#pragma unroll
        for (int m = 0; m < MT; ++m)
#pragma unroll
            for (int n = 0; n < 2; ++n)
#pragma unroll
                for (int e = 0; e < 4; ++e) acc[m][n][e] = 0.f;
        const uint32_t wbase = smem_u32(Wsm), dbase = smem_u32(Dsm);
#pragma unroll 2
        for (int ks = 0; ks < Q / 16; ++ks) {
            uint32_t bv[NH][4];
            const int brow = (lane & 7) + ((lane >> 4) << 3), bk = ks * 16 + ((lane >> 3) & 1) * 8;
#pragma unroll
            for (int h = 0; h < NH; ++h) ldsm_x4(dbase + h * S::DBYTES + swz<S::WP>(brow, bk), bv[h]);
#pragma unroll
            for (int m = 0; m < MT; ++m) {
                const int arow = (warp + 8 * m) * 16 + (lane & 15), ak = ks * 16 + (lane >> 4) * 8;
                uint32_t a[NH][4];
#pragma unroll
                for (int h = 0; h < NH; ++h) ldsm_x4(wbase + h * S::WBYTES + swz<S::WP>(arow, ak), a[h]);
#pragma unroll
                for (int n = 0; n < 2; ++n) {
                    if (NS != 1) {
                        mma_bf16(acc[m][n], a[0], bv[NH - 1][2 * n], bv[NH - 1][2 * n + 1]);
                        mma_bf16(acc[m][n], a[NH - 1], bv[0][2 * n], bv[0][2 * n + 1]);
                    }
                    mma_bf16(acc[m][n], a[0], bv[0][2 * n], bv[0][2 * n + 1]);
                }
            }
        }
        if (NS != 1 && s + 1 < T) load_step(s + 1);
        __syncthreads();
        cluster_wait();
#pragma unroll
        for (int m = 0; m < MT; ++m)
#pragma unroll
            for (int n = 0; n < 2; ++n)
#pragma unroll
                for (int e = 0; e < 4; e += 2) {
                    const int k = (warp + 8 * m) * 16 + (lane >> 2) + (e >= 2 ? 8 : 0);
                    const int bl = n * 8 + 2 * (lane & 3);
                    const int dst = k / U, x = xslot(k % U, bl);
                    const float2 v = make_float2(acc[m][n][e], acc[m][n][e + 1]);
                    if (dst == c) {
                        *reinterpret_cast<float2*>(own + x) = v;
                    } else {
                        const float* rs = recv + (c < dst ? c : c - 1) * NB * U + x;
                        st_cluster_v2_f32(mapa(smem_u32(rs), dst), v);
                    }
                }
        cluster_arrive();
        cluster_wait();
    }
#pragma unroll
    for (int i = 0; i < PAIRS; ++i) {
        const int p = tid + i * SCAN_THREADS, u = p % U, b = p / U, x = xslot(u, b);
        float v = dhz[i];
#pragma unroll
        for (int src = 0; src < CS; ++src) v += slot(src)[x];
        dhc[((int64_t)d * B + bt0 + b) * H + c * U + u] = v;
    }
}

}

static inline int64_t rup(int64_t v, int64_t m) { return (v + m - 1) / m * m; }
static inline int64_t tc_pack_elems(int64_t R, int64_t K, int64_t batch, int prec) {
    return (prec == BIGRU_PREC_BF16X3 ? 2 : 1) * batch * rup(R, htc::WG_BM) * rup(K, htc::WG_BK);
}
static inline int64_t tc_gemm_ws_elems(int64_t M, int64_t N, int64_t K, int64_t batch, int prec) {
    return tc_pack_elems(M, K, batch, prec) + tc_pack_elems(N, K, batch, prec);
}
static inline int wg_splits(int64_t tiles, int64_t kblocks) {
    const int64_t s = std::min(cdiv64(4 * 132, tiles), kblocks / 8);
    if (s <= 1) return 1;
    const int64_t per = cdiv64(kblocks, s);
    return (int)cdiv64(kblocks, per);
}

struct Planes {
    const htc::bf16_t* hi; const htc::bf16_t* lo;
    int64_t cols, rows, depth, pitch;
};

typedef CUresult (*PFN_encodeTiled_t)(CUtensorMap*, CUtensorMapDataType, cuuint32_t, void*, const cuuint64_t*, const cuuint64_t*,
                                      const cuuint32_t*, const cuuint32_t*, CUtensorMapInterleave, CUtensorMapSwizzle,
                                      CUtensorMapL2promotion, CUtensorMapFloatOOBfill);
static int make_plane_map(CUtensorMap* m, const htc::bf16_t* base, const Planes& p, bool mn) {
    static PFN_encodeTiled_t enc = nullptr;
    if (!enc) {
        void* f = nullptr;
        cudaDriverEntryPointQueryResult q;
        if (cudaGetDriverEntryPoint("cuTensorMapEncodeTiled", &f, cudaEnableDefault, &q) != cudaSuccess || q != cudaDriverEntryPointSuccess) {
            bigru_set_error("tc_gemm: cuTensorMapEncodeTiled is unavailable");
            return BIGRU_ERR_CUDA;
        }
        enc = (PFN_encodeTiled_t)f;
    }
    const cuuint64_t dims[3] = {(cuuint64_t)p.cols, (cuuint64_t)p.rows, (cuuint64_t)p.depth};
    const cuuint64_t strides[2] = {(cuuint64_t)p.pitch * 2, (cuuint64_t)(p.pitch * p.rows) * 2};
    const cuuint32_t box[3] = {64u, mn ? 64u : 128u, 1u}, es[3] = {1u, 1u, 1u};
    CUresult r = enc(m, CU_TENSOR_MAP_DATA_TYPE_BFLOAT16, 3, const_cast<htc::bf16_t*>(base), dims, strides, box, es,
                     CU_TENSOR_MAP_INTERLEAVE_NONE, CU_TENSOR_MAP_SWIZZLE_128B, CU_TENSOR_MAP_L2_PROMOTION_L2_256B,
                     CU_TENSOR_MAP_FLOAT_OOB_FILL_NONE);
    if (r != CUDA_SUCCESS) { bigru_set_error("tc_gemm: cuTensorMapEncodeTiled failed (%d)", (int)r); return BIGRU_ERR_CUDA; }
    return BIGRU_OK;
}

template <int NS, int AMN, int BMN>
static int wg_launch(const CUtensorMap (&tm)[4], const htc::WgJob& j, int grid, cudaStream_t st) {
    constexpr int STAGES = NS == 1 ? 4 : 3;
    const int smem = STAGES * 2 * (NS == 1 ? 1 : 2) * 16384 + 1024 + 2 * STAGES * 8;
    auto k = htc::wg_gemm_kernel<NS, STAGES, AMN, BMN>;
    CUDA_TRY(cudaFuncSetAttribute(k, cudaFuncAttributeMaxDynamicSharedMemorySize, smem));
    k<<<grid, 384, smem, st>>>(tm[0], tm[1], tm[2], tm[3], j);
    LAUNCH_CHECK();
    return BIGRU_OK;
}

static int wg_gemm(htc::WgJob j, const Planes& A, bool amn, const Planes& B, bool bmn, int prec, cudaStream_t st) {
    if (j.M <= 0 || j.N <= 0) return BIGRU_OK;
    const bool x3 = prec == BIGRU_PREC_BF16X3;
    if (x3 != (A.lo != nullptr) || x3 != (B.lo != nullptr) || amn != bmn) {
        bigru_set_error("tc_gemm: operand planes do not match the precision / majors");
        return BIGRU_ERR_ARG;
    }
    j.tm = (int)cdiv64(j.M, htc::WG_BM);
    j.tn = (int)cdiv64(j.N, htc::WG_BN);
    CUtensorMap tm[4];
    TRY(make_plane_map(&tm[0], A.hi, A, amn));
    TRY(make_plane_map(&tm[2], B.hi, B, bmn));
    if (x3) {
        TRY(make_plane_map(&tm[1], A.lo, A, amn));
        TRY(make_plane_map(&tm[3], B.lo, B, bmn));
    } else {
        tm[1] = tm[0]; tm[3] = tm[2];
    }
    int dev = 0, nsm = 132;
    CUDA_TRY(cudaGetDevice(&dev));
    CUDA_TRY(cudaDeviceGetAttribute(&nsm, cudaDevAttrMultiProcessorCount, dev));
    const int64_t units = (int64_t)j.tm * j.tn * j.batch * j.splits;
    const int grid = (int)std::min<int64_t>(units, nsm);
    const int rc = amn ? (x3 ? wg_launch<3, 1, 1>(tm, j, grid, st) : wg_launch<1, 1, 1>(tm, j, grid, st))
                       : (x3 ? wg_launch<3, 0, 0>(tm, j, grid, st) : wg_launch<1, 0, 0>(tm, j, grid, st));
    TRY(rc);
    if (j.splits > 1) {
        const int64_t n = (int64_t)j.batch * j.M * j.N;
        htc::splitk_reduce_kernel<<<(unsigned)std::min<int64_t>(cdiv64(n, 256), 132 * 8), 256, 0, st>>>(j.part, j.splits, j.batch, j.M,
                                                                                                        j.N, j.C, j.ldc, j.zC, j.beta);
        LAUNCH_CHECK();
    }
    return BIGRU_OK;
}

static htc::WgJob wg_job(float* C, int M, int N, int64_t ldc, int batch, int64_t kblocks) {
    htc::WgJob j{};
    j.C = C; j.M = M; j.N = N; j.ldc = ldc; j.batch = batch; j.kblocks = (int)kblocks; j.kbd = (int)kblocks; j.splits = 1;
    return j;
}

static int tc_pack(const float* src, int64_t s_r, int64_t s_k, int64_t zsrc, int R, int K, int batch, int prec, htc::bf16_t* ws,
                   Planes* out, cudaStream_t st) {
    const bool x3 = prec == BIGRU_PREC_BF16X3;
    const int Rp = (int)rup(R, htc::WG_BM), Kp = (int)rup(K, htc::WG_BK);
    const int64_t sz = (int64_t)batch * Rp * Kp;
    *out = Planes{ws, x3 ? ws + sz : nullptr, Kp, Rp, batch, Kp};
    KLAUNCH(KC_PACK, 0.0, (4.0 + (x3 ? 4.0 : 2.0)) * batch * (double)R * K, st,
            htc::tc_pack_kernel<<<dim3(Kp / 32, Rp / 32, batch), dim3(32, 8), 0, st>>>(src, s_r, s_k, zsrc, R, K, Rp, Kp, ws,
                                                                                     x3 ? ws + sz : nullptr));
    return BIGRU_OK;
}

static int tc_gemm_launch(const GemmArgs& g, int prec, int cls, htc::bf16_t* ws, cudaStream_t st) {
    if (g.M <= 0 || g.N <= 0 || g.K <= 0) return BIGRU_OK;
    if (g.splitk != 1 || g.mask_period) {
        bigru_set_error("tc_gemm_launch: split-K and row masks are not supported");
        return BIGRU_ERR_ARG;
    }
    Planes A, B;
    TRY(tc_pack(g.A, g.sam, g.sak, g.zA, g.M, g.K, g.batch, prec, ws, &A, st));
    TRY(tc_pack(g.B, g.sbn, g.sbk, g.zB, g.N, g.K, g.batch, prec, ws + tc_pack_elems(g.M, g.K, g.batch, prec), &B, st));
    ProfScope ps(cls, 2.0 * g.M * g.N * (double)g.K * g.batch, 0.0, st);
    htc::WgJob j = wg_job(g.C, g.M, g.N, g.ldc, g.batch, cdiv64(g.K, htc::WG_BK));
    j.bias = g.bias; j.beta = g.beta; j.zC = g.zC; j.zBias = g.zBias;
    j.a.zsel = 1; j.b.zsel = 1;
    return wg_gemm(j, A, false, B, false, prec, st);
}

template <typename... KArgs, typename... Args>
static int launch_cluster(void (*kernel)(KArgs...), int cs, int ntiles, int D, int smem, cudaStream_t st, Args... args) {
    CUDA_TRY(cudaFuncSetAttribute(kernel, cudaFuncAttributeMaxDynamicSharedMemorySize, smem));
    cudaLaunchConfig_t cfg{};
    cfg.gridDim = dim3(cs, ntiles, D);
    cfg.blockDim = dim3(htc::SCAN_THREADS);
    cfg.dynamicSmemBytes = smem;
    cfg.stream = st;
    cudaLaunchAttribute attr[1];
    attr[0].id = cudaLaunchAttributeClusterDimension;
    attr[0].val.clusterDim.x = cs; attr[0].val.clusterDim.y = 1; attr[0].val.clusterDim.z = 1;
    cfg.attrs = attr; cfg.numAttrs = 1;
    CUDA_TRY(cudaLaunchKernelEx(&cfg, kernel, args...));
    return BIGRU_OK;
}

template <int HH, int NS, bool LEN>
static int scan_fwd_launch(int out, int cs, int nt, int D, cudaStream_t st, const float* gi, const float* Whh, const float* bhh,
                           int64_t zW, const float* h0, float* Y, float* G, float* hn, htc::bf16_t* yh, htc::bf16_t* yl, int B, int T,
                           const int* len) {
    constexpr int smem = htc::FwdSmem<HH, NS>::TOTAL;
    switch (out) {
        case htc::SCAN_TRAIN:
            return launch_cluster(htc::gru_scan_fwd_kernel<HH, NS, htc::SCAN_TRAIN, LEN>, cs, nt, D, smem, st, gi, Whh, bhh, zW, h0, Y, G, hn, yh, yl, B, T, D, len);
        case htc::SCAN_INFER_LOWER:
            return launch_cluster(htc::gru_scan_fwd_kernel<HH, NS, htc::SCAN_INFER_LOWER, LEN>, cs, nt, D, smem, st, gi, Whh, bhh, zW, h0, Y, G, hn, yh, yl, B, T, D, len);
        case htc::SCAN_INFER_TOP:
            return launch_cluster(htc::gru_scan_fwd_kernel<HH, NS, htc::SCAN_INFER_TOP, LEN>, cs, nt, D, smem, st, gi, Whh, bhh, zW, h0, Y, G, hn, yh, yl, B, T, D, len);
    }
    bigru_set_error("tc_scan_fwd: no kernel writes this set of outputs (Y %d, G %d, planes %d)", Y != nullptr, G != nullptr, yh != nullptr);
    return BIGRU_ERR_ARG;
}

static int tc_scan_fwd(const bigru_plan& p, int l, const float* gi, const float* Whh, const float* bhh, const float* h0,
                       float* Y, float* G, float* hn, htc::bf16_t* yh, htc::bf16_t* yl, const int* len, cudaStream_t st) {
    const int H = p.H, D = p.D, B = p.B, T = p.T, cs = H / htc::SCAN_U, nt = B / htc::SCAN_NB;
    const int64_t zW = p.ld_block(l);
    const int out = (Y ? htc::SCAN_Y : 0) | (G ? htc::SCAN_G : 0) | (yh ? htc::SCAN_PLANES : 0);
    ProfScope ps(KC_TC_SCAN_FWD, 2.0 * D * B * (double)T * 3 * H * H, 0.0, st);
#define FWD(HH, NS) return len ? scan_fwd_launch<HH, NS, true>(out, cs, nt, D, st, gi, Whh, bhh, zW, h0, Y, G, hn, yh, yl, B, T, len) \
                               : scan_fwd_launch<HH, NS, false>(out, cs, nt, D, st, gi, Whh, bhh, zW, h0, Y, G, hn, yh, yl, B, T, len)
    if (p.prec == BIGRU_PREC_BF16X3) {
        if (H == 128) FWD(128, 3);
        if (H == 256) FWD(256, 3);
    } else {
        if (H == 128) FWD(128, 1);
        if (H == 256) FWD(256, 1);
        if (H == 512) FWD(512, 1);
    }
#undef FWD
    bigru_set_error("tc_scan_fwd: no kernel for H=%d at precision %d", H, p.prec);
    return BIGRU_ERR_UNSUPPORTED;
}

static int tc_scan_bwd(const bigru_plan& p, int l, const float* G, const float* Y, const float* h0, const float* dY, float* dhc,
                       float* dgi, float* dgh, const float* Whh, htc::bf16_t* gih, htc::bf16_t* gil, htc::bf16_t* ghh,
                       htc::bf16_t* ghl, const int* len, cudaStream_t st) {
    const int H = p.H, D = p.D, B = p.B, T = p.T, cs = H / htc::SCAN_U, nt = B / htc::SCAN_NB;
    const int64_t zW = p.ld_block(l);
    ProfScope ps(KC_TC_SCAN_BWD, 2.0 * D * B * (double)T * 3 * H * H, 0.0, st);
#define BWD(HH, NS) return len ? launch_cluster(htc::gru_scan_bwd_kernel<HH, NS, true>, cs, nt, D, htc::BwdSmem<HH, NS>::TOTAL, st, G, Y, h0, dY, dhc, dgi, dgh, Whh, zW, gih, gil, ghh, ghl, B, T, D, len) \
                           : launch_cluster(htc::gru_scan_bwd_kernel<HH, NS, false>, cs, nt, D, htc::BwdSmem<HH, NS>::TOTAL, st, G, Y, h0, dY, dhc, dgi, dgh, Whh, zW, gih, gil, ghh, ghl, B, T, D, len)
    if (p.prec == BIGRU_PREC_BF16X3) {
        if (H == 128) BWD(128, 3);
        if (H == 256) BWD(256, 3);
    } else {
        if (H == 128) BWD(128, 1);
        if (H == 256) BWD(256, 1);
        if (H == 512) BWD(512, 1);
    }
#undef BWD
    bigru_set_error("tc_scan_bwd: no kernel for H=%d at precision %d", H, p.prec);
    return BIGRU_ERR_UNSUPPORTED;
}
```

### include/bigru_b200.h

```cpp
#ifndef BIGRU_B200_H
#define BIGRU_B200_H

#include <stddef.h>
#include <stdint.h>

#ifdef __cplusplus
extern "C" {
#endif

#define BIGRU_OK               0
#define BIGRU_ERR_ARG         -1
#define BIGRU_ERR_CUDA        -2
#define BIGRU_ERR_DEVICE      -3
#define BIGRU_ERR_UNSUPPORTED -4

#define BIGRU_PREC_FP32 0
#define BIGRU_PREC_BF16 1
#define BIGRU_PREC_BF16X3 2

#define BIGRU_LOSS_CE   0
#define BIGRU_LOSS_BCE  1
#define BIGRU_LOSS_MLSM 2

typedef struct bigru_plan bigru_plan;

const char* bigru_last_error(void);
int  bigru_version(void);
int  bigru_device_check(int dev);

int  bigru_plan_create(int B, int T, int F, int H, int L, int C, int bidirectional, int precision,
                       bigru_plan** out);
int  bigru_plan_destroy(bigru_plan* plan);
int64_t bigru_param_count(const bigru_plan* plan);
int  bigru_param_offset(const bigru_plan* plan, int layer, int dir, int which,
                        int64_t* offset, int64_t* rows, int64_t* cols);
int  bigru_workspace_bytes(const bigru_plan* plan, size_t* stash_bytes, size_t* scratch_bytes);

int  bigru_stash_argmax_offset(const bigru_plan* plan, size_t* byte_offset);
int  bigru_stash_output_offset(const bigru_plan* plan, int layer, size_t* byte_offset);
#define BIGRU_WS_GATES       0
#define BIGRU_WS_Y_PLANES    1
#define BIGRU_WS_IN_PLANES   2
#define BIGRU_WS_DGI         3
#define BIGRU_WS_DGH         4
#define BIGRU_WS_DGI_PLANES  5
#define BIGRU_WS_DGH_PLANES  6
#define BIGRU_WS_DY          7
#define BIGRU_WS_DHC         8
#define BIGRU_WS_DCAT        9
#define BIGRU_WS_COUNT      10
int  bigru_workspace_region(const bigru_plan* plan, int which, int layer, int* in_scratch, size_t* byte_offset,
                            size_t* lo_byte_offset, int64_t* pitch);

int  bigru_forward(const bigru_plan* plan, const float* d_params, const float* d_x, const float* d_h0,
                   float dropout_p, int spatial, int training, uint64_t seed,
                   void* d_stash, void* d_scratch, float* d_logits, float* d_hn, void* stream);

int  bigru_infer_workspace_bytes(const bigru_plan* plan, size_t* bytes);
int  bigru_infer(const bigru_plan* plan, const float* d_params, const float* d_x, const float* d_h0,
                 void* d_workspace, float* d_logits, void* stream);

int  bigru_forward_lengths(const bigru_plan* plan, const float* d_params, const float* d_x, const float* d_h0,
                           float dropout_p, int spatial, int training, uint64_t seed,
                           void* d_stash, void* d_scratch, float* d_logits, float* d_hn, const int32_t* d_lengths,
                           void* stream);
int  bigru_infer_lengths(const bigru_plan* plan, const float* d_params, const float* d_x, const float* d_h0,
                         void* d_workspace, float* d_logits, const int32_t* d_lengths, void* stream);
int  bigru_backward_lengths(const bigru_plan* plan, const float* d_params, const float* d_x, const float* d_h0,
                            float dropout_p, int spatial, int training, uint64_t seed,
                            const void* d_stash, void* d_scratch, const float* d_dlogits,
                            float* d_grads, float* d_dx, float* d_dh0, const int32_t* d_lengths, void* stream);

int  bigru_backward(const bigru_plan* plan, const float* d_params, const float* d_x, const float* d_h0,
                    float dropout_p, int spatial, int training, uint64_t seed,
                    const void* d_stash, void* d_scratch, const float* d_dlogits,
                    float* d_grads, float* d_dx, float* d_dh0, void* stream);

int  bigru_loss(int kind, const float* d_logits, const void* d_target, const float* d_weight,
                const float* d_pos_weight, int B, int C, double denom, float* d_loss,
                float* d_dlogits, void* stream);

#define BIGRU_SQNORM_WS 528
int  bigru_sqnorm(const float* d_g, int64_t n, float* d_out, float* d_ws, void* stream);
int  bigru_adam_tick(int* d_step, float* d_sqnorm, void* stream);
int  bigru_clip_adam_step_dev(float* d_params, float* d_grads, float* d_m, float* d_v, int64_t n,
                              const float* d_sqnorm, float clip, float lr, float b1, float b2, float eps,
                              const int* d_step, float grad_scale, void* stream);

int  bigru_window_gather_norm(const float* d_src, const float* d_xmin, const float* d_xmax,
                              int64_t start, int64_t N, int B, int T, int F, float* d_out, void* stream);
int  bigru_window_targets(const float* d_y, int64_t start, int64_t N, int B, int T, int C,
                          float* d_out, void* stream);

int  bigru_chunk_minmax(const float* d_table, int64_t N, int F, int64_t row_lo, int64_t row_hi, float* d_min,
                        float* d_max, void* stream);

int  bigru_window_features(const float* d_close, const float* d_high, const float* d_low, const float* d_volume,
                           const float* d_delta, int64_t n, const int* vol_periods, int n_vol, const int* price_periods,
                           int n_price, const int* delta_periods, int n_delta, int bb_period, float bb_std,
                           int stochastic, float n1, float n2, float* d_out, float* d_targets, int* n_out, void* stream);

int  bigru_infer_window(const float* d_params, const float* d_x, const float* d_xmin, const float* d_xmax, int B, int T,
                        int F, int H, int L, int C, int bidirectional, float* d_logits, float* d_probs, void* stream);

int  bigru_multilabel_counts(const float* d_logits, const float* d_target, int B, int C,
                             long long* d_counts, void* stream);

long long   bigru_launch_count(void);
void        bigru_launch_count_add(long long n);
int         bigru_prof_enable(int on);
int         bigru_prof_classes(void);
const char* bigru_prof_class_name(int cls);
int         bigru_prof_report(int cls, double* ms, long long* launches, double* flops, double* bytes);

#ifdef __cplusplus
}
#endif
#endif
```

Before: 45510.

## Balance GRU scan cluster waves with double-width batch tiles and residency-aware geometry

The forward scan kernel can now process either a single or a double batch tile per cluster. It uses one h buffer with an empty-barrier handshake when the tile is doubled. The launch queries how many clusters can be resident and picks how many tiles get doubled, so the last partial wave disappears. The backward scan also gets a split of the tail work, L8, based on residency. This is meant to remove wave-quantization idle time, at the cost of extra peer synchronization and more register pressure for the wider tiles.

```diff
diff --git a/financial_market_data_analysis_b200/_lib.py b/financial_market_data_analysis_b200/_lib.py
--- a/financial_market_data_analysis_b200/_lib.py
+++ b/financial_market_data_analysis_b200/_lib.py
@@ -26,6 +26,7 @@
     "bigru_stash_argmax_offset": (_i, [_vp, C.POINTER(C.c_size_t)]),
     "bigru_stash_output_offset": (_i, [_vp, _i, C.POINTER(C.c_size_t)]),
     "bigru_workspace_region": (_i, [_vp, _i, _i, C.POINTER(_i), C.POINTER(C.c_size_t), C.POINTER(C.c_size_t), C.POINTER(_i64)]),
+    "bigru_scan_geometry": (_i, [_vp, _i, C.POINTER(_i), C.POINTER(_i)]),
     "bigru_forward": (_i, [_vp, _vp, _vp, _vp, _f, _i, _i, _u64, _vp, _vp, _vp, _vp, _vp]),
     "bigru_backward": (_i, [_vp, _vp, _vp, _vp, _f, _i, _i, _u64, _vp, _vp, _vp, _vp, _vp, _vp, _vp]),
     "bigru_infer_workspace_bytes": (_i, [_vp, C.POINTER(C.c_size_t)]),
diff --git a/financial_market_data_analysis_b200/csrc/api.cu b/financial_market_data_analysis_b200/csrc/api.cu
--- a/financial_market_data_analysis_b200/csrc/api.cu
+++ b/financial_market_data_analysis_b200/csrc/api.cu
@@ -16,7 +16,7 @@
 }
 
 extern "C" const char* bigru_last_error(void) { return g_err; }
-extern "C" int bigru_version(void) { return 207; }
+extern "C" int bigru_version(void) { return 208; }
 
 extern "C" int bigru_device_check(int dev) {
     int n = 0;
@@ -229,6 +229,16 @@
 extern "C" int bigru_stash_output_offset(const bigru_plan* p, int layer, size_t* byte_offset) {
     if (!p || !byte_offset || layer < 0 || layer >= p->L) { bigru_set_error("stash_output_offset: bad argument"); return BIGRU_ERR_ARG; }
     *byte_offset = (size_t)stash_layout(*p).Y[layer] * sizeof(float);
+    return BIGRU_OK;
+}
+
+extern "C" int bigru_scan_geometry(const bigru_plan* p, int scan, int* R, int* n_split) {
+    if (!p || !R || !n_split || (scan != 0 && scan != 1)) { bigru_set_error("scan_geometry: bad argument"); return BIGRU_ERR_ARG; }
+    if (p->prec == BIGRU_PREC_FP32) { bigru_set_error("scan_geometry: BIGRU_PREC_FP32 runs no cluster scans"); return BIGRU_ERR_UNSUPPORTED; }
+    int geom[2] = {0, 0};
+    if (scan == 0) TRY(tc_scan_fwd(*p, 0, nullptr, nullptr, nullptr, nullptr, nullptr, nullptr, nullptr, nullptr, nullptr, nullptr, 0, geom));
+    else TRY(tc_scan_bwd(*p, 0, nullptr, nullptr, nullptr, nullptr, nullptr, nullptr, nullptr, nullptr, nullptr, nullptr, nullptr, nullptr, nullptr, 0, geom));
+    *R = geom[0]; *n_split = geom[1];
     return BIGRU_OK;
 }
 
diff --git a/financial_market_data_analysis_b200/csrc/tc_hopper.cuh b/financial_market_data_analysis_b200/csrc/tc_hopper.cuh
--- a/financial_market_data_analysis_b200/csrc/tc_hopper.cuh
+++ b/financial_market_data_analysis_b200/csrc/tc_hopper.cuh
@@ -2,6 +2,8 @@
 #include "common.cuh"
 #include "kernels_f32.cuh"
 #include <algorithm>
+#include <map>
+#include <mutex>
 #include <cuda.h>
 #include <cuda_bf16.h>
 
@@ -302,32 +304,52 @@
 template <int H, int NS>
 struct FwdSmem {
     static constexpr int NH = NS == 1 ? 1 : 2;
+    static constexpr int NBMAX = NS == 1 ? SCAN_NB : 2 * SCAN_NB;
+    static constexpr int NBUF = NBMAX == SCAN_NB ? 2 : 1;
     static constexpr int WP = H * 2;
     static constexpr int WBYTES = 3 * SCAN_U * WP;
-    static constexpr int HBYTES = SCAN_NB * H * 2;
-    static constexpr int SLICE = SCAN_NB * SCAN_U * 2;
-    static constexpr int TOTAL = NH * WBYTES + 2 * NH * HBYTES + 2 * 8;
+    static constexpr int HBYTES = NBMAX * H * 2;
+    static constexpr int SLICE = NBMAX * SCAN_U * 2;
+    static constexpr int TOTAL = NH * WBYTES + NBUF * NH * HBYTES + 2 * 8;
 };
 
+__device__ __forceinline__ void scan_tile(int q, int m2, int ntd, int D, int& d, int& bt0, int& nb) {
+    if (q < D * m2) {
+        d = q / m2; bt0 = (q % m2) * 2 * SCAN_NB; nb = 2 * SCAN_NB;
+    } else {
+        const int r = q - D * m2, o = ntd - 2 * m2;
+        d = r / o; bt0 = (2 * m2 + r % o) * SCAN_NB; nb = SCAN_NB;
+    }
+}
+
+template <int NBMAX>
 __device__ __forceinline__ uint32_t hsw(int b, int k) {
-    return (uint32_t)((k / SCAN_U) * (SCAN_NB * SCAN_U * 2)) + swz<SCAN_U * 2>(b, k % SCAN_U);
-}
-
-template <int H, int NS, int OUT, bool LEN>
-__global__ void __launch_bounds__(SCAN_THREADS, 1)
-gru_scan_fwd_kernel(const float* __restrict__ gi, const float* __restrict__ Whh, const float* __restrict__ bhh, int64_t zW,
-                    const float* __restrict__ h0, float* __restrict__ Y, float* __restrict__ G, float* __restrict__ hn_out,
-                    bf16_t* __restrict__ yh, bf16_t* __restrict__ yl, int B, int T, int D, const int* __restrict__ lens) {
+    return (uint32_t)((k / SCAN_U) * (NBMAX * SCAN_U * 2)) + swz<SCAN_U * 2>(b, k % SCAN_U);
+}
+
+__device__ __forceinline__ void mbar_arrive_peer(uint64_t* bar, uint32_t cta) {
+    asm volatile("mbarrier.arrive.release.cluster.shared::cluster.b64 _, [%0];" ::"r"(mapa(smem_u32(bar), cta)) : "memory");
+}
+
+template <int H, int NS, int OUT, bool LEN, int JN>
+__device__ __forceinline__ void gru_scan_fwd_tile(const float* __restrict__ gi, const float* __restrict__ Whh,
+                                                  const float* __restrict__ bhh, int64_t zW, const float* __restrict__ h0,
+                                                  float* __restrict__ Y, float* __restrict__ G, float* __restrict__ hn_out,
+                                                  bf16_t* __restrict__ yh, bf16_t* __restrict__ yl, int B, int T, int D,
+                                                  const int* __restrict__ lens, int d, int bt0) {
     using S = FwdSmem<H, NS>;
-    constexpr int U = SCAN_U, CS = H / U, NH = S::NH;
-    static_assert(SCAN_THREADS % (SCAN_NB * (U / 8)) == 0, "a thread copies the same Y plane row in every pass");
+    constexpr int U = SCAN_U, CS = H / U, NH = S::NH, JMAX = JN, jn = JN, nb = JN * SCAN_NB;
+    constexpr int NBMAX = nb, NBUF = S::NBUF * S::NBMAX / nb;
+    constexpr int HBYTES = nb * H * 2, SLICE = nb * U * 2;
+    static_assert(NBUF * HBYTES == S::NBUF * S::HBYTES, "both tile sizes fill the h region");
+    static_assert(SCAN_THREADS % (nb * (U / 8)) == 0, "a thread copies the same Y plane row in every pass");
     extern __shared__ __align__(128) uint8_t smem[];
     uint8_t* Wsm = smem;
     uint8_t* Hsm = smem + NH * S::WBYTES;
-    uint64_t* full = reinterpret_cast<uint64_t*>(Hsm + 2 * NH * S::HBYTES);
-    const int c = (int)cluster_rank(), tile = blockIdx.y, d = blockIdx.z;
+    uint64_t* full = reinterpret_cast<uint64_t*>(Hsm + NBUF * NH * HBYTES);
+    uint64_t* empty = full + 1;
+    const int c = (int)cluster_rank();
     const int tid = threadIdx.x, lane = tid & 31, warp = tid >> 5;
-    const int bt0 = tile * SCAN_NB;
     const float* W = Whh + d * zW;
 
     for (int i = tid; i < 3 * U * H; i += SCAN_THREADS) {
@@ -338,122 +360,149 @@
         *reinterpret_cast<bf16_t*>(Wsm + swz<S::WP>(q, k)) = hi;
         if (NH == 2) *reinterpret_cast<bf16_t*>(Wsm + S::WBYTES + swz<S::WP>(q, k)) = lo;
     }
-    for (int i = tid; i < SCAN_NB * H; i += SCAN_THREADS) {
+    for (int i = tid; i < nb * H; i += SCAN_THREADS) {
         const int b = i / H, k = i % H;
         const float v = h0 ? h0[((int64_t)d * B + bt0 + b) * H + k] : 0.f;
         bf16_t hi, lo;
         split_bf16(v, hi, lo);
-        *reinterpret_cast<bf16_t*>(Hsm + hsw(b, k)) = hi;
-        if (NH == 2) *reinterpret_cast<bf16_t*>(Hsm + S::HBYTES + hsw(b, k)) = lo;
+        *reinterpret_cast<bf16_t*>(Hsm + hsw<NBMAX>(b, k)) = hi;
+        if (NH == 2) *reinterpret_cast<bf16_t*>(Hsm + HBYTES + hsw<NBMAX>(b, k)) = lo;
     }
     if (tid == 0) {
         mbar_init(full, 1);
-        mbar_init(full + 1, 1);
+        mbar_init(full + 1, NBUF == 2 ? 1 : CS - 1);
         asm volatile("fence.mbarrier_init.release.cluster;" ::: "memory");
     }
 
     const int ug = warp >> 1, nt = warp & 1;
-    int unit[2], bcol[2];
+    int unit[2], bcol[JMAX][2];
     unit[0] = ug * 16 + (lane >> 2); unit[1] = unit[0] + 8;
-    bcol[0] = nt * 8 + 2 * (lane & 3); bcol[1] = bcol[0] + 1;
-    float bias[3][2], hp[4];
+#pragma unroll
+    for (int j = 0; j < JMAX; ++j) {
+        bcol[j][0] = (nt * jn + j) * 8 + 2 * (lane & 3); bcol[j][1] = bcol[j][0] + 1;
+    }
+    float bias[3][2], hp[JMAX][4];
 #pragma unroll
     for (int gte = 0; gte < 3; ++gte)
 #pragma unroll
-        for (int j = 0; j < 2; ++j) bias[gte][j] = bhh[d * zW + gte * H + c * U + unit[j]];
-#pragma unroll
-    for (int e = 0; e < 4; ++e) {
-        const int b = bt0 + bcol[e & 1], j = c * U + unit[e >> 1];
-        hp[e] = h0 ? h0[((int64_t)d * B + b) * H + j] : 0.f;
-    }
-    int len[2] = {T, T}, rlen = T;
-    if (LEN) {
-        len[0] = lens[bt0 + bcol[0]]; len[1] = lens[bt0 + bcol[1]];
-        rlen = lens[bt0 + (tid / (U / 8)) % SCAN_NB];
-    }
+        for (int i = 0; i < 2; ++i) bias[gte][i] = bhh[d * zW + gte * H + c * U + unit[i]];
+    int len[JMAX][2], rlen = T;
+#pragma unroll
+    for (int j = 0; j < JMAX; ++j) {
+#pragma unroll
+        for (int e = 0; e < 4; ++e) {
+            const int b = bt0 + bcol[j][e & 1], k = c * U + unit[e >> 1];
+            hp[j][e] = h0 ? h0[((int64_t)d * B + b) * H + k] : 0.f;
+        }
+        len[j][0] = len[j][1] = T;
+        if (LEN) { len[j][0] = lens[bt0 + bcol[j][0]]; len[j][1] = lens[bt0 + bcol[j][1]]; }
+    }
+    if (LEN) rlen = lens[bt0 + (tid / (U / 8)) % nb];
     cluster_arrive();
     cluster_wait();
 
     const int DH = D * H;
     for (int s = 0; s < T; ++s) {
         const int t = d == 0 ? s : T - 1 - s;
-        const int buf = s & 1;
-        if (s > 0) mbar_wait<true>(full + buf, ((s - 1) >> 1) & 1);
-        if (tid == 0 && s + 1 < T) mbar_arrive_expect_tx(full + (buf ^ 1), (CS - 1) * NH * S::SLICE);
-        float giv[3][4];
-#pragma unroll
-        for (int e = 0; e < 4; ++e) {
-            const int64_t row = (int64_t)(bt0 + bcol[e & 1]) * T + t;
-            const float* gr = gi + ((int64_t)d * B * T + row) * 3 * H + c * U + unit[e >> 1];
-#pragma unroll
-            for (int gte = 0; gte < 3; ++gte) giv[gte][e] = gr[gte * H];
-        }
-        float acc[3][4];
+        const int buf = NBUF == 2 ? s & 1 : 0, nbuf = NBUF == 2 ? buf ^ 1 : 0;
+        if (s > 0) mbar_wait<true>(full + buf, (NBUF == 2 ? (s - 1) >> 1 : s - 1) & 1);
+        if (tid == 0 && s + 1 < T) mbar_arrive_expect_tx(full + nbuf, (CS - 1) * NH * nb * U * 2);
+        float giv[3][JMAX][4];
+#pragma unroll
+        for (int j = 0; j < JMAX; ++j)
+#pragma unroll
+            for (int e = 0; e < 4; ++e) {
+                const int64_t row = (int64_t)(bt0 + bcol[j][e & 1]) * T + t;
+                const float* gr = gi + ((int64_t)d * B * T + row) * 3 * H + c * U + unit[e >> 1];
+#pragma unroll
+                for (int gte = 0; gte < 3; ++gte) giv[gte][j][e] = gr[gte * H];
+            }
+        float acc[3][JMAX][4];
 #pragma unroll
         for (int gte = 0; gte < 3; ++gte)
 #pragma unroll
-            for (int e = 0; e < 4; ++e) acc[gte][e] = 0.f;
-        const uint32_t hbase = smem_u32(Hsm + buf * NH * S::HBYTES);
+            for (int j = 0; j < JMAX; ++j)
+#pragma unroll
+                for (int e = 0; e < 4; ++e) acc[gte][j][e] = 0.f;
+        const uint32_t hbase = smem_u32(Hsm + buf * NH * HBYTES);
         const uint32_t wbase = smem_u32(Wsm);
 #pragma unroll 4
         for (int ks = 0; ks < H / 16; ++ks) {
-            uint32_t bh[NH][2];
-            const int brow = nt * 8 + (lane & 7), bk = ks * 16 + ((lane >> 3) & 1) * 8;
-#pragma unroll
-            for (int h = 0; h < NH; ++h) ldsm_x2(hbase + h * S::HBYTES + hsw(brow, bk), bh[h]);
+            uint32_t bh[JMAX][NH][2];
+            const int bk = ks * 16 + ((lane >> 3) & 1) * 8;
+#pragma unroll
+            for (int j = 0; j < JMAX; ++j)
+#pragma unroll
+                for (int h = 0; h < NH; ++h)
+                    ldsm_x2(hbase + h * HBYTES + hsw<NBMAX>((nt * jn + j) * 8 + (lane & 7), bk), bh[j][h]);
 #pragma unroll
             for (int gte = 0; gte < 3; ++gte) {
                 const int arow = gte * U + ug * 16 + (lane & 15), ak = ks * 16 + (lane >> 4) * 8;
                 uint32_t a[NH][4];
 #pragma unroll
                 for (int h = 0; h < NH; ++h) ldsm_x4(wbase + h * S::WBYTES + swz<S::WP>(arow, ak), a[h]);
-                if (NS != 1) {
-                    mma_bf16(acc[gte], a[0], bh[NH - 1][0], bh[NH - 1][1]);
-                    mma_bf16(acc[gte], a[NH - 1], bh[0][0], bh[0][1]);
+#pragma unroll
+                for (int j = 0; j < JMAX; ++j) {
+                    if (NS != 1) {
+                        mma_bf16(acc[gte][j], a[0], bh[j][NH - 1][0], bh[j][NH - 1][1]);
+                        mma_bf16(acc[gte][j], a[NH - 1], bh[j][0][0], bh[j][0][1]);
+                    }
+                    mma_bf16(acc[gte][j], a[0], bh[j][0][0], bh[j][0][1]);
                 }
-                mma_bf16(acc[gte], a[0], bh[0][0], bh[0][1]);
-            }
-        }
-        const int nbuf = buf ^ 1;
-#pragma unroll
-        for (int e = 0; e < 4; ++e) {
-            const int b = bt0 + bcol[e & 1], ul = unit[e >> 1], j = c * U + ul;
-            const float r = sigmoid_f(giv[0][e] + acc[0][e] + bias[0][e >> 1]);
-            const float z = sigmoid_f(giv[1][e] + acc[1][e] + bias[1][e >> 1]);
-            const float hnv = acc[2][e] + bias[2][e >> 1];
-            const float n = tanhf(giv[2][e] + r * hnv);
-            const bool pad = LEN && t >= len[e & 1];
-            const float h = pad ? hp[e] : (1.f - z) * n + z * hp[e];
-            hp[e] = h;
-            const int64_t row = (int64_t)b * T + t;
-            if (OUT & SCAN_Y) Y[row * DH + d * H + j] = pad ? 0.f : h;
-            if ((OUT & SCAN_G) && !pad) {
-                float* gs = G + ((int64_t)d * B * T + row) * 4 * H + j;
-                gs[0] = r; gs[H] = z; gs[2 * H] = n; gs[3 * H] = hnv;
-            }
-            if (hn_out && s == T - 1) hn_out[((int64_t)d * B + b) * H + j] = h;
-            bf16_t hi, lo;
-            split_bf16(h, hi, lo);
-            uint8_t* la = Hsm + nbuf * NH * S::HBYTES + hsw(bcol[e & 1], j);
-            *reinterpret_cast<bf16_t*>(la) = hi;
-            if (NH == 2) *reinterpret_cast<bf16_t*>(la + S::HBYTES) = lo;
-        }
+            }
+        }
+        if (NBUF == 1) {
+            __syncthreads();
+            if (tid < CS - 1) mbar_arrive_peer(empty, (c + 1 + tid) % CS);
+        }
+        float hv[JMAX][4];
+#pragma unroll
+        for (int j = 0; j < JMAX; ++j)
+#pragma unroll
+            for (int e = 0; e < 4; ++e) {
+                const int b = bt0 + bcol[j][e & 1], ul = unit[e >> 1], k = c * U + ul;
+                const float r = sigmoid_f(giv[0][j][e] + acc[0][j][e] + bias[0][e >> 1]);
+                const float z = sigmoid_f(giv[1][j][e] + acc[1][j][e] + bias[1][e >> 1]);
+                const float hnv = acc[2][j][e] + bias[2][e >> 1];
+                const float n = tanhf(giv[2][j][e] + r * hnv);
+                const bool pad = LEN && t >= len[j][e & 1];
+                const float h = pad ? hp[j][e] : (1.f - z) * n + z * hp[j][e];
+                hp[j][e] = h;
+                hv[j][e] = h;
+                const int64_t row = (int64_t)b * T + t;
+                if (OUT & SCAN_Y) Y[row * DH + d * H + k] = pad ? 0.f : h;
+                if ((OUT & SCAN_G) && !pad) {
+                    float* gs = G + ((int64_t)d * B * T + row) * 4 * H + k;
+                    gs[0] = r; gs[H] = z; gs[2 * H] = n; gs[3 * H] = hnv;
+                }
+                if (hn_out && s == T - 1) hn_out[((int64_t)d * B + b) * H + k] = h;
+            }
+        if (NBUF == 1) mbar_wait<true>(empty, s & 1);
+#pragma unroll
+        for (int j = 0; j < JMAX; ++j)
+#pragma unroll
+            for (int e = 0; e < 4; ++e) {
+                bf16_t hi, lo;
+                split_bf16(hv[j][e], hi, lo);
+                uint8_t* la = Hsm + nbuf * NH * HBYTES + hsw<NBMAX>(bcol[j][e & 1], c * U + unit[e >> 1]);
+                *reinterpret_cast<bf16_t*>(la) = hi;
+                if (NH == 2) *reinterpret_cast<bf16_t*>(la + HBYTES) = lo;
+            }
         asm volatile("fence.proxy.async.shared::cta;" ::: "memory");
         __syncthreads();
-        const uint32_t own = smem_u32(Hsm + nbuf * NH * S::HBYTES + c * S::SLICE);
+        const uint32_t own = smem_u32(Hsm + nbuf * NH * HBYTES + c * SLICE);
         if (tid == 0 && s + 1 < T) {
 #pragma unroll
             for (int p = 1; p < CS; ++p) {
                 const uint32_t dst = (c + p) % CS;
 #pragma unroll
-                for (int h = 0; h < NH; ++h) bulk_copy_to_peer(own + h * S::HBYTES, S::SLICE, full + nbuf, dst);
+                for (int h = 0; h < NH; ++h) bulk_copy_to_peer(own + h * HBYTES, nb * U * 2, full + nbuf, dst);
             }
         }
         if (OUT & SCAN_PLANES) {
-            for (int i = tid; i < NH * SCAN_NB * (U / 8); i += SCAN_THREADS) {
-                const int h = i / (SCAN_NB * U / 8), r = (i / (U / 8)) % SCAN_NB, kl = (i % (U / 8)) * 8;
-                uint4 v = *reinterpret_cast<const uint4*>(Hsm + nbuf * NH * S::HBYTES + h * S::HBYTES + c * S::SLICE +
-                                                          swz<U * 2>(r, kl));
+            for (int i = tid; i < NH * nb * (U / 8); i += SCAN_THREADS) {
+                const int h = i / (nb * U / 8), r = (i / (U / 8)) % nb, kl = (i % (U / 8)) * 8;
+                uint4 v = *reinterpret_cast<const uint4*>(Hsm + (nbuf * NH + h) * HBYTES + c * SLICE + swz<U * 2>(r, kl));
                 if (LEN && t >= rlen) v = make_uint4(0u, 0u, 0u, 0u);
                 *reinterpret_cast<uint4*>((h ? yl : yh) + ((int64_t)(bt0 + r) * T + t) * DH + d * H + c * U + kl) = v;
             }
@@ -461,6 +510,22 @@
     }
     cluster_arrive();
     cluster_wait();
+}
+
+template <int H, int NS, int OUT, bool LEN>
+__global__ void __launch_bounds__(SCAN_THREADS, 1)
+gru_scan_fwd_kernel(const float* __restrict__ gi, const float* __restrict__ Whh, const float* __restrict__ bhh, int64_t zW,
+                    const float* __restrict__ h0, float* __restrict__ Y, float* __restrict__ G, float* __restrict__ hn_out,
+                    bf16_t* __restrict__ yh, bf16_t* __restrict__ yl, int B, int T, int D, int m2, const int* __restrict__ lens) {
+    int d, bt0, nb;
+    scan_tile(blockIdx.y, m2, B / SCAN_NB, D, d, bt0, nb);
+    if constexpr (FwdSmem<H, NS>::NBMAX == 2 * SCAN_NB) {
+        if (nb == 2 * SCAN_NB) {
+            gru_scan_fwd_tile<H, NS, OUT, LEN, 2>(gi, Whh, bhh, zW, h0, Y, G, hn_out, yh, yl, B, T, D, lens, d, bt0);
+            return;
+        }
+    }
+    gru_scan_fwd_tile<H, NS, OUT, LEN, 1>(gi, Whh, bhh, zW, h0, Y, G, hn_out, yh, yl, B, T, D, lens, d, bt0);
 }
 
 template <int H, int NS>
@@ -481,23 +546,24 @@
     return kl * SCAN_NB + (((b >> 1) ^ g) << 1) + (b & 1);
 }
 
-template <int H, int NS, bool LEN>
-__global__ void __launch_bounds__(SCAN_THREADS, 1)
-gru_scan_bwd_kernel(const float* __restrict__ G, const float* __restrict__ Y, const float* __restrict__ h0,
-                    const float* __restrict__ dY, float* __restrict__ dhc, float* __restrict__ dgi, float* __restrict__ dgh,
-                    const float* __restrict__ Whh, int64_t zW, bf16_t* __restrict__ gih, bf16_t* __restrict__ gil,
-                    bf16_t* __restrict__ ghh, bf16_t* __restrict__ ghl, int B, int T, int D, const int* __restrict__ lens) {
+template <int H, int NS, bool LEN, int NR>
+__device__ __forceinline__ void gru_scan_bwd_tile(const float* __restrict__ G, const float* __restrict__ Y,
+                                                  const float* __restrict__ h0, const float* __restrict__ dY,
+                                                  float* __restrict__ dhc, float* __restrict__ dgi, float* __restrict__ dgh,
+                                                  const float* __restrict__ Whh, int64_t zW, bf16_t* __restrict__ gih,
+                                                  bf16_t* __restrict__ gil, bf16_t* __restrict__ ghh, bf16_t* __restrict__ ghl,
+                                                  int B, int T, int D, const int* __restrict__ lens, int d, int bt0) {
     using S = BwdSmem<H, NS>;
     constexpr int U = SCAN_U, CS = H / U, NH = S::NH, Q = S::Q, NB = SCAN_NB;
     constexpr int MT = H / 16 / 8;
-    constexpr int PAIRS = NB * U / SCAN_THREADS;
+    constexpr int PAIRS = NR * U / SCAN_THREADS;
+    constexpr int NBLK = NR / 8;
     extern __shared__ __align__(128) uint8_t smem[];
     uint8_t* Wsm = smem;
     uint8_t* Dsm = smem + NH * S::WBYTES;
     float* recv = reinterpret_cast<float*>(Dsm + NH * S::DBYTES);
-    const int c = (int)cluster_rank(), tile = blockIdx.y, d = blockIdx.z;
+    const int c = (int)cluster_rank();
     const int tid = threadIdx.x, lane = tid & 31, warp = tid >> 5;
-    const int bt0 = tile * NB;
     const float* W = Whh + d * zW;
     float* own = reinterpret_cast<float*>(Dsm);
     auto slot = [&](int src) -> float* { return src == c ? own : recv + (src < c ? src : src - 1) * NB * U; };
@@ -587,8 +653,8 @@
         }
         if (NS == 1 && s + 1 < T) load_step(s + 1);
         __syncthreads();
-        for (int i = tid; i < NH * NB * (Q / 8); i += SCAN_THREADS) {
-            const int h = i / (NB * Q / 8), r = (i / (Q / 8)) % NB, q = (i % (Q / 8)) * 8, gte = q / U;
+        for (int i = tid; i < NH * NR * (Q / 8); i += SCAN_THREADS) {
+            const int h = i / (NR * Q / 8), r = (i / (Q / 8)) % NR, q = (i % (Q / 8)) * 8, gte = q / U;
             uint4 v = *reinterpret_cast<const uint4*>(Dsm + h * S::DBYTES + swz<S::WP>(r, q));
             const int64_t o = ((int64_t)d * B * T + (int64_t)(bt0 + r) * T + t) * 3 * H + gte * H + c * U + q % U;
             if (gte < 2) *reinterpret_cast<uint4*>((h ? gil : gih) + o) = v;
@@ -599,7 +665,7 @@
 #pragma unroll
         for (int m = 0; m < MT; ++m)
 #pragma unroll
-            for (int n = 0; n < 2; ++n)
+            for (int n = 0; n < NBLK; ++n)
 #pragma unroll
                 for (int e = 0; e < 4; ++e) acc[m][n][e] = 0.f;
         const uint32_t wbase = smem_u32(Wsm), dbase = smem_u32(Dsm);
@@ -616,7 +682,7 @@
 #pragma unroll
                 for (int h = 0; h < NH; ++h) ldsm_x4(wbase + h * S::WBYTES + swz<S::WP>(arow, ak), a[h]);
 #pragma unroll
-                for (int n = 0; n < 2; ++n) {
+                for (int n = 0; n < NBLK; ++n) {
                     if (NS != 1) {
                         mma_bf16(acc[m][n], a[0], bv[NH - 1][2 * n], bv[NH - 1][2 * n + 1]);
                         mma_bf16(acc[m][n], a[NH - 1], bv[0][2 * n], bv[0][2 * n + 1]);
@@ -631,7 +697,7 @@
 #pragma unroll
         for (int m = 0; m < MT; ++m)
 #pragma unroll
-            for (int n = 0; n < 2; ++n)
+            for (int n = 0; n < NBLK; ++n)
 #pragma unroll
                 for (int e = 0; e < 4; e += 2) {
                     const int k = (warp + 8 * m) * 16 + (lane >> 2) + (e >= 2 ? 8 : 0);
@@ -658,6 +724,23 @@
     }
 }
 
+template <int H, int NS, bool LEN>
+__global__ void __launch_bounds__(SCAN_THREADS, 1)
+gru_scan_bwd_kernel(const float* __restrict__ G, const float* __restrict__ Y, const float* __restrict__ h0,
+                    const float* __restrict__ dY, float* __restrict__ dhc, float* __restrict__ dgi, float* __restrict__ dgh,
+                    const float* __restrict__ Whh, int64_t zW, bf16_t* __restrict__ gih, bf16_t* __restrict__ gil,
+                    bf16_t* __restrict__ ghh, bf16_t* __restrict__ ghl, int B, int T, int D, int L8, const int* __restrict__ lens) {
+    const int ntd = B / SCAN_NB, n16 = D * ntd - L8, q = blockIdx.y;
+    if (q < n16) {
+        gru_scan_bwd_tile<H, NS, LEN, SCAN_NB>(G, Y, h0, dY, dhc, dgi, dgh, Whh, zW, gih, gil, ghh, ghl, B, T, D, lens, q / ntd,
+                                                (q % ntd) * SCAN_NB);
+    } else {
+        const int f = n16 + (q - n16) / 2;
+        gru_scan_bwd_tile<H, NS, LEN, SCAN_NB / 2>(G, Y, h0, dY, dhc, dgi, dgh, Whh, zW, gih, gil, ghh, ghl, B, T, D, lens,
+                                                    f / ntd, (f % ntd) * SCAN_NB + ((q - n16) & 1) * (SCAN_NB / 2));
+    }
+}
+
 }
 
 static inline int64_t rup(int64_t v, int64_t m) { return (v + m - 1) / m * m; }
@@ -783,47 +866,97 @@
     return wg_gemm(j, A, false, B, false, prec, st);
 }
 
-template <typename... KArgs, typename... Args>
-static int launch_cluster(void (*kernel)(KArgs...), int cs, int ntiles, int D, int smem, cudaStream_t st, Args... args) {
-    CUDA_TRY(cudaFuncSetAttribute(kernel, cudaFuncAttributeMaxDynamicSharedMemorySize, smem));
+template <typename K>
+static cudaLaunchConfig_t cluster_config(K kernel, int cs, int ny, int nz, int smem, cudaStream_t st, cudaLaunchAttribute* attr) {
     cudaLaunchConfig_t cfg{};
-    cfg.gridDim = dim3(cs, ntiles, D);
+    cfg.gridDim = dim3(cs, ny, nz);
     cfg.blockDim = dim3(htc::SCAN_THREADS);
     cfg.dynamicSmemBytes = smem;
     cfg.stream = st;
-    cudaLaunchAttribute attr[1];
     attr[0].id = cudaLaunchAttributeClusterDimension;
     attr[0].val.clusterDim.x = cs; attr[0].val.clusterDim.y = 1; attr[0].val.clusterDim.z = 1;
     cfg.attrs = attr; cfg.numAttrs = 1;
+    return cfg;
+}
+
+template <typename... KArgs, typename... Args>
+static int launch_cluster(void (*kernel)(KArgs...), int cs, int ny, int nz, int smem, cudaStream_t st, Args... args) {
+    CUDA_TRY(cudaFuncSetAttribute(kernel, cudaFuncAttributeMaxDynamicSharedMemorySize, smem));
+    cudaLaunchAttribute attr[1];
+    const cudaLaunchConfig_t cfg = cluster_config(kernel, cs, ny, nz, smem, st, attr);
     CUDA_TRY(cudaLaunchKernelEx(&cfg, kernel, args...));
     return BIGRU_OK;
 }
 
+template <typename... KArgs>
+static int cluster_residency(void (*kernel)(KArgs...), int cs, int smem, int* R) {
+    static std::mutex mu;
+    static std::map<std::pair<const void*, int>, int> cache;
+    int dev = 0;
+    CUDA_TRY(cudaGetDevice(&dev));
+    const std::pair<const void*, int> key((const void*)kernel, dev);
+    {
+        std::lock_guard<std::mutex> g(mu);
+        const auto it = cache.find(key);
+        if (it != cache.end()) { *R = it->second; return BIGRU_OK; }
+    }
+    CUDA_TRY(cudaFuncSetAttribute(kernel, cudaFuncAttributeMaxDynamicSharedMemorySize, smem));
+    cudaLaunchAttribute attr[1];
+    const cudaLaunchConfig_t cfg = cluster_config(kernel, cs, 1, 1, smem, 0, attr);
+    int n = 0;
+    CUDA_TRY(cudaOccupancyMaxActiveClusters(&n, (void*)kernel, &cfg));
+    if (n <= 0) { bigru_set_error("scan: no %d-CTA cluster with %d bytes of shared memory fits on this device", cs, smem); return BIGRU_ERR_DEVICE; }
+    {
+        std::lock_guard<std::mutex> g(mu);
+        cache[key] = n;
+    }
+    *R = n;
+    return BIGRU_OK;
+}
+
+static void scan_geometry(int R, bool two, int B, int D, int* m2, int* clusters) {
+    const int ntd = B / htc::SCAN_NB, n = D * ntd;
+    int n2 = 0;
+    if (two) {
+        const int rounds = (n + 2 * R - 1) / (2 * R);
+        n2 = std::max(0, n - rounds * R);
+        n2 = std::min((n2 + D - 1) / D * D, D * (ntd / 2));
+    }
+    *m2 = n2 / D;
+    *clusters = n - n2;
+}
+
 template <int HH, int NS, bool LEN>
-static int scan_fwd_launch(int out, int cs, int nt, int D, cudaStream_t st, const float* gi, const float* Whh, const float* bhh,
-                           int64_t zW, const float* h0, float* Y, float* G, float* hn, htc::bf16_t* yh, htc::bf16_t* yl, int B, int T,
-                           const int* len) {
+static int scan_fwd_launch(int out, int cs, int B, int D, cudaStream_t st, const float* gi, const float* Whh, const float* bhh,
+                           int64_t zW, const float* h0, float* Y, float* G, float* hn, htc::bf16_t* yh, htc::bf16_t* yl, int T,
+                           const int* len, int* geom) {
     constexpr int smem = htc::FwdSmem<HH, NS>::TOTAL;
+    void (*k)(const float*, const float*, const float*, int64_t, const float*, float*, float*, float*, htc::bf16_t*, htc::bf16_t*,
+              int, int, int, int, const int*) = nullptr;
     switch (out) {
-        case htc::SCAN_TRAIN:
-            return launch_cluster(htc::gru_scan_fwd_kernel<HH, NS, htc::SCAN_TRAIN, LEN>, cs, nt, D, smem, st, gi, Whh, bhh, zW, h0, Y, G, hn, yh, yl, B, T, D, len);
-        case htc::SCAN_INFER_LOWER:
-            return launch_cluster(htc::gru_scan_fwd_kernel<HH, NS, htc::SCAN_INFER_LOWER, LEN>, cs, nt, D, smem, st, gi, Whh, bhh, zW, h0, Y, G, hn, yh, yl, B, T, D, len);
-        case htc::SCAN_INFER_TOP:
-            return launch_cluster(htc::gru_scan_fwd_kernel<HH, NS, htc::SCAN_INFER_TOP, LEN>, cs, nt, D, smem, st, gi, Whh, bhh, zW, h0, Y, G, hn, yh, yl, B, T, D, len);
-    }
-    bigru_set_error("tc_scan_fwd: no kernel writes this set of outputs (Y %d, G %d, planes %d)", Y != nullptr, G != nullptr, yh != nullptr);
-    return BIGRU_ERR_ARG;
+        case htc::SCAN_TRAIN: k = htc::gru_scan_fwd_kernel<HH, NS, htc::SCAN_TRAIN, LEN>; break;
+        case htc::SCAN_INFER_LOWER: k = htc::gru_scan_fwd_kernel<HH, NS, htc::SCAN_INFER_LOWER, LEN>; break;
+        case htc::SCAN_INFER_TOP: k = htc::gru_scan_fwd_kernel<HH, NS, htc::SCAN_INFER_TOP, LEN>; break;
+        default:
+            bigru_set_error("tc_scan_fwd: no kernel writes this set of outputs (Y %d, G %d, planes %d)", Y != nullptr, G != nullptr, yh != nullptr);
+            return BIGRU_ERR_ARG;
+    }
+    int R = 0, m2 = 0, clusters = 0;
+    TRY(cluster_residency(k, cs, smem, &R));
+    scan_geometry(R, htc::FwdSmem<HH, NS>::NBMAX == 2 * htc::SCAN_NB, B, D, &m2, &clusters);
+    if (geom) { geom[0] = R; geom[1] = D * m2; return BIGRU_OK; }
+    ProfScope ps(KC_TC_SCAN_FWD, 2.0 * D * B * (double)T * 3 * HH * HH, 0.0, st);
+    return launch_cluster(k, cs, clusters, 1, smem, st, gi, Whh, bhh, zW, h0, Y, G, hn, yh, yl, B, T, D, m2, len);
 }
 
 static int tc_scan_fwd(const bigru_plan& p, int l, const float* gi, const float* Whh, const float* bhh, const float* h0,
-                       float* Y, float* G, float* hn, htc::bf16_t* yh, htc::bf16_t* yl, const int* len, cudaStream_t st) {
-    const int H = p.H, D = p.D, B = p.B, T = p.T, cs = H / htc::SCAN_U, nt = B / htc::SCAN_NB;
+                       float* Y, float* G, float* hn, htc::bf16_t* yh, htc::bf16_t* yl, const int* len, cudaStream_t st,
+                       int* geom = nullptr) {
+    const int H = p.H, D = p.D, B = p.B, T = p.T, cs = H / htc::SCAN_U;
     const int64_t zW = p.ld_block(l);
-    const int out = (Y ? htc::SCAN_Y : 0) | (G ? htc::SCAN_G : 0) | (yh ? htc::SCAN_PLANES : 0);
-    ProfScope ps(KC_TC_SCAN_FWD, 2.0 * D * B * (double)T * 3 * H * H, 0.0, st);
-#define FWD(HH, NS) return len ? scan_fwd_launch<HH, NS, true>(out, cs, nt, D, st, gi, Whh, bhh, zW, h0, Y, G, hn, yh, yl, B, T, len) \
-                               : scan_fwd_launch<HH, NS, false>(out, cs, nt, D, st, gi, Whh, bhh, zW, h0, Y, G, hn, yh, yl, B, T, len)
+    const int out = geom ? htc::SCAN_TRAIN : (Y ? htc::SCAN_Y : 0) | (G ? htc::SCAN_G : 0) | (yh ? htc::SCAN_PLANES : 0);
+#define FWD(HH, NS) return len ? scan_fwd_launch<HH, NS, true>(out, cs, B, D, st, gi, Whh, bhh, zW, h0, Y, G, hn, yh, yl, T, len, geom) \
+                               : scan_fwd_launch<HH, NS, false>(out, cs, B, D, st, gi, Whh, bhh, zW, h0, Y, G, hn, yh, yl, T, len, geom)
     if (p.prec == BIGRU_PREC_BF16X3) {
         if (H == 128) FWD(128, 3);
         if (H == 256) FWD(256, 3);
@@ -837,14 +970,33 @@
     return BIGRU_ERR_UNSUPPORTED;
 }
 
+static void scan_bwd_geometry(int R, int B, int D, int* L8, int* clusters) {
+    const int n = D * (B / htc::SCAN_NB), rounds = (n + R - 1) / R, L = n - (rounds - 1) * R;
+    *L8 = rounds > 1 && 2 * L <= R ? L : 0;
+    *clusters = n + *L8;
+}
+
+template <int HH, int NS, bool LEN>
+static int scan_bwd_launch(int cs, int B, int D, cudaStream_t st, const float* G, const float* Y, const float* h0, const float* dY,
+                           float* dhc, float* dgi, float* dgh, const float* Whh, int64_t zW, htc::bf16_t* gih, htc::bf16_t* gil,
+                           htc::bf16_t* ghh, htc::bf16_t* ghl, int T, const int* len, int* geom) {
+    constexpr int smem = htc::BwdSmem<HH, NS>::TOTAL;
+    auto k = htc::gru_scan_bwd_kernel<HH, NS, LEN>;
+    int R = 0, L8 = 0, clusters = 0;
+    TRY(cluster_residency(k, cs, smem, &R));
+    scan_bwd_geometry(R, B, D, &L8, &clusters);
+    if (geom) { geom[0] = R; geom[1] = L8; return BIGRU_OK; }
+    ProfScope ps(KC_TC_SCAN_BWD, 2.0 * D * B * (double)T * 3 * HH * HH, 0.0, st);
+    return launch_cluster(k, cs, clusters, 1, smem, st, G, Y, h0, dY, dhc, dgi, dgh, Whh, zW, gih, gil, ghh, ghl, B, T, D, L8, len);
+}
+
 static int tc_scan_bwd(const bigru_plan& p, int l, const float* G, const float* Y, const float* h0, const float* dY, float* dhc,
                        float* dgi, float* dgh, const float* Whh, htc::bf16_t* gih, htc::bf16_t* gil, htc::bf16_t* ghh,
-                       htc::bf16_t* ghl, const int* len, cudaStream_t st) {
-    const int H = p.H, D = p.D, B = p.B, T = p.T, cs = H / htc::SCAN_U, nt = B / htc::SCAN_NB;
+                       htc::bf16_t* ghl, const int* len, cudaStream_t st, int* geom = nullptr) {
+    const int H = p.H, D = p.D, B = p.B, T = p.T, cs = H / htc::SCAN_U;
     const int64_t zW = p.ld_block(l);
-    ProfScope ps(KC_TC_SCAN_BWD, 2.0 * D * B * (double)T * 3 * H * H, 0.0, st);
-#define BWD(HH, NS) return len ? launch_cluster(htc::gru_scan_bwd_kernel<HH, NS, true>, cs, nt, D, htc::BwdSmem<HH, NS>::TOTAL, st, G, Y, h0, dY, dhc, dgi, dgh, Whh, zW, gih, gil, ghh, ghl, B, T, D, len) \
-                           : launch_cluster(htc::gru_scan_bwd_kernel<HH, NS, false>, cs, nt, D, htc::BwdSmem<HH, NS>::TOTAL, st, G, Y, h0, dY, dhc, dgi, dgh, Whh, zW, gih, gil, ghh, ghl, B, T, D, len)
+#define BWD(HH, NS) return len ? scan_bwd_launch<HH, NS, true>(cs, B, D, st, G, Y, h0, dY, dhc, dgi, dgh, Whh, zW, gih, gil, ghh, ghl, T, len, geom) \
+                           : scan_bwd_launch<HH, NS, false>(cs, B, D, st, G, Y, h0, dY, dhc, dgi, dgh, Whh, zW, gih, gil, ghh, ghl, T, len, geom)
     if (p.prec == BIGRU_PREC_BF16X3) {
         if (H == 128) BWD(128, 3);
         if (H == 256) BWD(256, 3);
diff --git a/include/bigru_b200.h b/include/bigru_b200.h
--- a/include/bigru_b200.h
+++ b/include/bigru_b200.h
@@ -51,6 +51,8 @@
 #define BIGRU_WS_COUNT      10
 int  bigru_workspace_region(const bigru_plan* plan, int which, int layer, int* in_scratch, size_t* byte_offset,
                             size_t* lo_byte_offset, int64_t* pitch);
+
+int  bigru_scan_geometry(const bigru_plan* plan, int scan, int* R, int* n_split);
 
 int  bigru_forward(const bigru_plan* plan, const float* d_params, const float* d_x, const float* d_h0,
                    float dropout_p, int spatial, int training, uint64_t seed,
```

Result: faster. 48430, median of 6 (+6.4%).
